# saamiya225/Graph-and-sequential-recommendation-systems

Measured on AMD Instinct MI355X. Metric: BPR training steps/sec (one step = K-layer LightGCN propagation + BPR loss + backward + Adam on a global batch of 2048 triplets), higher is better.
Workload: dtype bf16 (activation storage; f32 accumulation, parameters, gradients and Adam); 1 GPU; gowalla: 29858 users x 40981 items, 810128 train interactions, nnz(A_hat)=1620256, layers=3, dim=64, bpr_batch=2048; global_batch=2048, per_gpu_batch=2048, scaling_mode=strong, multi_gpu_status=n/a, parallelism=single GPU, act_dtype=bf16, xcd_remap=1, row_order=xcd

## Files before the change

graph-and-sequential-recommendation-systems_amd/_lib.py:

```python
import ctypes as C
import os

from . import build as _build

F32, BF16, FP8 = 0, 1, 2
ABI_VERSION = 13
MAX_LAYERS = 8
MAX_NEG_RATIO = 16

LOSS_BPR, LOSS_SOFTMAX, LOSS_INBATCH = 0, 1, 2
LOSS_DIRECTAU = 4
SCORE_DOT, SCORE_COSINE = 0, 1

_c_i32p =C.POINTER(C.c_int32)
_c_i64p = C.POINTER(C.c_int64)
_c_f32p = C.POINTER(C.c_float)
_vp = C.c_void_p


def fp8_col_of_byte(d):
    import numpy as np
    b = np.arange(d)
    l, j, e = b // 16, (b % 16) // 4, b % 4
    return ((j * (d // 16) + l) * 4 + e).astype(np.int64)
# ... 65 lines not shown
    "lgcn_ctx_get_step": (C.c_int64, [_vp]),
    "lgcn_ctx_hub_rows": (C.c_int64, [_vp]),
    "lgcn_ctx_set_step": (None, [_vp, C.c_int64]),
    "lgcn_ctx_set_lr": (None, [_vp, C.c_double]),
    "lgcn_ctx_set_dp_local": (C.c_int, [_vp, C.c_int]),
    "lgcn_train_step": (C.c_int, [_vp, _vp, _vp, _vp, C.c_int32, _vp, _vp]),
    "lgcn_train_epoch": (C.c_int, [_vp, _vp, _vp, _vp, C.c_int64, C.c_int32, _vp, _vp]),
    "lgcn_apply_perm_multi": (C.c_int, [_vp, C.c_int, _vp, C.c_int64, _vp, _vp, _vp, C.c_int32, _vp]),
    "lgcn_train_step_multi": (C.c_int, [_vp, _vp, _vp, _vp, C.c_int64, C.c_int32, C.c_int32, _vp, _vp]),
    "lgcn_train_epoch_multi": (C.c_int, [_vp, _vp, _vp, _vp, C.c_int32, C.c_int64, C.c_int32, _vp, _vp]),
    "lgcn_ctx_set_loss": (C.c_int, [_vp, C.c_int32, C.c_float]),
    "lgcn_ctx_get_loss": (C.c_int32, [_vp, _vp]),
    "lgcn_train_step_inbatch": (C.c_int, [_vp, _vp, _vp, C.c_int32, _vp, _vp]),
    "lgcn_train_epoch_inbatch": (C.c_int, [_vp, _vp, _vp, C.c_int64, C.c_int32, _vp, _vp]),
    "lgcn_ctx_set_inbatch_scores": (C.c_int, [_vp, C.c_int, _vp]),
    "lgcn_ctx_get_inbatch_scores": (C.c_int, [_vp, C.POINTER(_vp)]),
    "lgcn_ctx_set_inbatch_mix": (C.c_int, [_vp, C.c_int32]),
    "lgcn_ctx_get_inbatch_mix": (C.c_int32, [_vp]),
    "lgcn_train_step_inbatch_mix": (C.c_int, [_vp, _vp, _vp, _vp, C.c_int64, C.c_int32, C.c_int32, _vp, _vp]),
    "lgcn_train_epoch_inbatch_mix": (C.c_int, [_vp, _vp, _vp, _vp, C.c_int32, C.c_int64, C.c_int32, _vp, _vp]),
    "lgcn_ctx_set_directau": (C.c_int, [_vp, C.c_float]),
    "lgcn_ctx_get_directau": (C.c_int, [_vp, _vp]),
    "lgcn_train_step_directau": (C.c_int, [_vp, _vp, _vp, C.c_int32, _vp, _vp]),
    "lgcn_train_epoch_directau": (C.c_int, [_vp, _vp, _vp, C.c_int64, C.c_int32, _vp, _vp]),
    "lgcn_ctx_set_hard_neg": (C.c_int, [_vp, C.c_int32, C.c_uint64, _vp]),
    "lgcn_ctx_get_hard_neg": (C.c_int32, [_vp]),
    "lgcn_hard_neg_rank": (C.c_uint32, [C.c_uint64, C.c_int64, C.c_int32, C.c_int32]),
    "lgcn_dp_block_floats": (C.c_int64, [_vp, C.c_int32, C.c_int32]),
    "lgcn_train_step_dp_part1": (C.c_int, [_vp, _vp, _vp, _vp, C.c_int32, C.c_int32, C.c_int32, _vp]),
    "lgcn_train_step_dp_dense_part1": (C.c_int, [_vp, _vp, _vp, _vp, C.c_int32, C.c_int32, C.c_int32, _vp]),
    "lgcn_ctx_gate_total": (C.c_int, [_vp, C.POINTER(C.c_void_p), C.POINTER(C.c_int32)]),
    "lgcn_train_step_dp_part2": (C.c_int, [_vp, _vp, _vp, _vp, C.c_int32, C.c_int32, _vp, _vp, _vp]),
    "lgcn_ctx_check": (C.c_int, [_vp, _vp]),
    "lgcn_eval_topk": (C.c_int, [_vp, C.c_int32, C.c_int32, C.c_int32, _vp, C.c_int32, _vp, _vp, C.c_int32, _vp, _vp, _vp]),
    "lgcn_eval_topk_masked": (C.c_int, [_vp, C.c_int32, C.c_int32, C.c_int32, _vp, C.c_int32, _vp, _vp, C.c_int32, _vp, _vp, _vp, _vp]),
    "lgcn_eval_mask_words": (C.c_int64, [C.c_int32, C.c_int32]),
    "lgcn_eval_build_masks": (C.c_int, [_vp, C.c_int32, _vp, _vp, C.c_int32, _vp, _vp]),
    "lgcn_eval_topk_fp32": (C.c_int, [_vp, C.c_int32, C.c_int32, C.c_int32, _vp, C.c_int32, _vp, _vp, C.c_int32, _vp, _vp, _vp]),
    "lgcn_eval_metrics": (C.c_int, [_vp, C.c_int32, C.c_int32, _vp, _vp, _vp, C.c_int32, _vp, _vp, _vp]),
    "lgcn_eval_kmax": (C.c_int32, []),
    "lgcn_eval_topk_ex": (C.c_int, [_vp, C.c_int32, C.c_int32, C.c_int32, _vp, C.c_int32, _vp, _vp, _vp, C.c_int32, _vp, _vp,
                                    C.c_int64, C.c_int32, _vp]),
    "lgcn_eval_metrics_ex": (C.c_int, [_vp, C.c_int32, C.c_int32, _vp, _vp, _vp, C.c_int32, _vp, _vp, _vp]),
    "lgcn_eval_ranks": (C.c_int, [_vp, C.c_int32, C.c_int32, C.c_int32, _vp, C.c_int32, _vp, _vp, _vp, _vp, C.c_int64, _vp, _vp, _vp,
                                  C.c_int32, _vp]),
    "lgcn_eval_rank_metrics": (C.c_int, [C.c_int32, C.c_int32, _vp, _vp, _vp, _vp, _vp, C.c_int64, _vp, _vp, _vp, _vp, C.c_int32,
                                         _vp, _vp, _vp]),
    "lgcn_i2i_topk": (C.c_int, [_vp, _vp, C.c_int64, C.c_int64, C.c_int32, C.c_int32, C.c_int32, C.c_int32, _vp, _vp, _vp, _vp]),
    "lgcn_i2i_finish": (C.c_int, [_vp, _vp, _vp, C.c_int32, C.c_int32, C.c_int64, _vp, _vp, _vp, C.POINTER(C.c_int64), _vp]),
    "lgcn_dp_available": (C.c_int, []),
    "lgcn_dp_unique_id": (C.c_int, [_vp]),
    "lgcn_dp_init": (C.c_int, [_vp, C.c_int, C.c_int, C.POINTER(_vp)]),
    "lgcn_train_step_i64": (C.c_int, [_vp, _vp, _vp, _vp, C.c_int32, _vp, _vp, _vp]),
    "lgcn_train_step_cols_part1": (C.c_int, [_vp, _vp, _vp, _vp, C.c_int32, C.POINTER(_vp), _vp]),
    "lgcn_train_step_cols_part2": (C.c_int, [_vp, _vp, _vp, _vp, C.c_int32, _vp, _vp]),
    "lgcn_dp_allreduce_sum_f32": (C.c_int, [_vp, _vp, C.c_int64, _vp]),
    "lgcn_dp_init_loopback": (C.c_int, [C.c_int, C.POINTER(_vp)]),
    "lgcn_dp_destroy": (None, [_vp]),
    "lgcn_dp_world": (C.c_int, [_vp]),
    "lgcn_dp_rank": (C.c_int, [_vp]),
    "lgcn_train_epoch_dp": (C.c_int, [_vp, _vp, _vp, _vp, _vp, C.c_int64, C.c_int32, C.c_int32, _vp, _vp, _vp, _vp]),
    "lgcn_rs_phase": (C.c_int, [_vp, C.c_int32, C.c_int32, _vp, _vp, _vp, C.c_int32, C.c_int32, C.c_int32, _vp, _vp, _vp]),
    "lgcn_rs_buffer": (C.c_int, [_vp, C.c_int32, C.c_int32, C.POINTER(_vp), C.POINTER(C.c_int32)]),
    "lgcn_ctx_set_dropout": (C.c_int, [_vp, C.c_float, C.c_uint64]),
    "lgcn_ctx_set_layer_weights": (C.c_int, [_vp, _vp, C.c_int32]),
    "lgcn_ctx_get_layer_weights": (C.c_int32, [_vp, _vp]),
    "lgcn_propagate_weighted": (C.c_int, [_vp, _vp, C.c_int, C.c_int, C.c_int, _vp, _vp, _vp, _vp]),
    "lgcn_dropout_mask": (C.c_int, [_vp, _vp, C.c_int64, C.c_int64, C.c_float, C.c_uint64, C.c_int64, _vp, _vp]),
    "lgcn_spmm_csr_drop": (C.c_int, [_vp, _vp, C.c_int, _vp, C.c_int, C.c_int, C.c_float, C.c_uint64, C.c_int64, C.c_int, _vp]),
    "lgcn_mf_create": (C.c_int, [C.POINTER(MfConfig), C.POINTER(_vp)]),
    "lgcn_mf_destroy": (None, [_vp]),
    "lgcn_mf_get_step": (C.c_int64, [_vp]),
    "lgcn_mf_set_step": (None, [_vp, C.c_int64]),
    "lgcn_mf_set_lr": (None, [_vp, C.c_double]),
    "lgcn_mf_train_step": (C.c_int, [_vp, _vp, _vp, _vp, C.c_int32, _vp, _vp]),
    "lgcn_mf_train_epoch": (C.c_int, [_vp, _vp, _vp, _vp, C.c_int64, C.c_int32, _vp, _vp]),
    "lgcn_mf_check": (C.c_int, [_vp, _vp]),
    "lgcn_ctx_set_fold_g32": (C.c_int, [_vp, C.c_int]),
    "lgcn_ctx_folded_steps": (C.c_int64, [_vp]),
    "lgcn_ctx_copy_arrivals": (C.c_int, [_vp, _vp, C.c_int64]),
    "lgcn_slot_multiplicity": (C.c_int, [_vp, _vp, _vp, C.c_int64, C.c_int32, C.c_int32, C.c_int64, _vp, _vp]),
    "lgcn_ctx_set_store_policy": (C.c_int, [_vp, C.c_int]),
    "lgcn_ctx_get_store_policy": (C.c_int, [_vp, _c_i32p]),
}

STORE_ADAM, STORE_XLAST = 1, 2
STORE_ARG_MV, STORE_ARG_P, STORE_ARG_Y = 1, 2, 4

_LIB = None


class LgcnError(RuntimeError):
    pass


def load():
    global _LIB
    if _LIB is not None:
        return _LIB
    path = _build.LIB_PATH
    if os.environ.get("LGCN_LIB_PATH"):
        pass
    elif _build.is_stale():
        if _build.must_not_build():
            if not os.path.exists(path):
                raise LgcnError(
                    f"liblgcn_hip.so is missing at {path}; this process is a distributed rank or runs under a "
                    "profiler and will not compile it. Build it first (__graft_entry__.build()).")
        elif _build.find_hipcc() is not None:
            _build.build()
        elif not os.path.exists(path):
            raise LgcnError(
                f"liblgcn_hip.so is missing at {path} and hipcc is not available to build it. "
                "The MI355X HIP library is the product path; there is no CPU fallback.")
    try:
        lib = C.CDLL(path)
    except OSError as e:
        raise LgcnError(f"cannot load {path}: {e}") from e
    for name, (res, args) in SIGNATURES.items():
        try:
            fn = getattr(lib, name)
        except AttributeError as e:
            raise LgcnError(f"{path} does not export {name} (stale build?)") from e
        fn.restype, fn.argtypes = res, args
    if lib.lgcn_abi_version() != ABI_VERSION:
        raise LgcnError("liblgcn_hip.so ABI version mismatch")
    _LIB = lib
    return lib


def check(rc, what=""):
    if rc != 0:
        msg = load().lgcn_last_error()
        raise LgcnError(f"{what} failed (rc={rc}): {msg.decode() if msg else ''}")


def npp(a):
    return a.ctypes.data_as(_vp)


def tp(t):
    return _vp(t.data_ptr()) if t is not None else _vp(0)


def require_gpu():
    import torch
    if not torch.cuda.is_available() or not load().lgcn_device_available():
        raise LgcnError("no MI355X/HIP device visible: the LightGCN HIP kernels cannot run "
                        "(there is deliberately no CPU fallback)")


def current_stream():
    import torch
    return _vp(torch.cuda.current_stream().cuda_stream)


EVAL_FP32 = 1


def eval_kmax():
    return int(load().lgcn_eval_kmax())


def _want(t, name, dtype, shape, dev=None):
    import torch
    if not torch.is_tensor(t):
        raise ValueError(f"{name} must be a tensor")
    if t.dtype != dtype:
# ... 321 lines not shown
```

graph-and-sequential-recommendation-systems_amd/csrc/lgcn_device.hip:

```cpp
#include <hip/hip_runtime.h>
#include <stdint.h>
#include <stdio.h>
#include <math.h>

#include "lgcn_device_common.h"

typedef __attribute__((ext_vector_type(8))) float f32x8;
typedef __attribute__((ext_vector_type(4))) __bf16 bf16x4;
typedef __attribute__((ext_vector_type(8))) __bf16 bf16x8;
typedef __attribute__((ext_vector_type(16))) float f32x16;
typedef __attribute__((ext_vector_type(16))) __bf16 bf16x16;
typedef __attribute__((ext_vector_type(4))) uint32_t u32x4;
typedef __attribute__((ext_vector_type(2))) float f32x2;
struct fp8_t { uint8_t v; };
__host__ __device__ __forceinline__ int fp8_byte_of_col(int c, int D) { const int L = D / 16, q = c >> 2; return (q % L) * 16 + 4 * (q / L) + (c & 3); }
__device__ __forceinline__ const float *fp8_scales(const void *tab, int64_t n_rows, int D) { return (const float *)((const char *)tab + n_rows * D); }
__device__ __forceinline__ float *fp8_scales(void *tab, int64_t n_rows, int D) { return (float *)((char *)tab + n_rows * D); }

template <int C> struct VecF;
template <> struct VecF<4> { typedef f32x4 T; typedef bf16x4 B; };
template <> struct VecF<8> { typedef f32x8 T; typedef bf16x8 B; };
template <> struct VecF<16> { typedef f32x16 T; typedef bf16x16 B; };

template <int C> __device__ __forceinline__ typename VecF<C>::T zerov() {
    typename VecF<C>::T z;
#pragma unroll
    for (int i = 0; i < C; i++) z[i] = 0.f;
    return z;
}
template <int C> __device__ __forceinline__ typename VecF<C>::T loadv(const float *p) {
    return *reinterpret_cast<const typename VecF<C>::T *>(p);
}
template <int C> __device__ __forceinline__ typename VecF<C>::T loadv(const bf16_t *p) {
    return __builtin_convertvector(*reinterpret_cast<const typename VecF<C>::B *>(p), typename VecF<C>::T);
}
template <int C> __device__ __forceinline__ void storev(float *p, typename VecF<C>::T v) {
    *reinterpret_cast<typename VecF<C>::T *>(p) = v;
}
template <int C> __device__ __forceinline__ void storev(bf16_t *p, typename VecF<C>::T v) {
    *reinterpret_cast<typename VecF<C>::B *>(p) = __builtin_convertvector(v, typename VecF<C>::B);
}
__device__ __forceinline__ f32x4 load4(const float *p) { return loadv<4>(p); }
__device__ __forceinline__ f32x4 load4(const bf16_t *p) { return loadv<4>(p); }
__device__ __forceinline__ void store4(float *p, f32x4 v) { storev<4>(p, v); }
__device__ __forceinline__ void store4(bf16_t *p, f32x4 v) { storev<4>(p, v); }
template <int OFF> __device__ __forceinline__ void store16_wt(void *p, f32x4 v) {
    static_assert(OFF >= 0 && OFF < 4096 && OFF % 16 == 0, "immediate offset of a global store");
    asm volatile("global_store_dwordx4 %0, %1, off offset:%2 sc1\n\ts_nop 1" : : "v"(p), "v"(v), "n"(OFF) : "memory");
}
template <int C> __device__ __forceinline__ void storev_wt(float *p, typename VecF<C>::T v) {
    store16_wt<0>(p, f32x4{v[0], v[1], v[2], v[3]});
    if constexpr (C >= 8) store16_wt<16>(p, f32x4{v[4], v[5], v[6], v[7]});
    if constexpr (C == 16) { store16_wt<32>(p, f32x4{v[8], v[9], v[10], v[11]}); store16_wt<48>(p, f32x4{v[12], v[13], v[14], v[15]}); }
}
__device__ __forceinline__ void storev_wt(bf16_t *p, f32x8 v) {
    union { bf16x8 b; f32x4 f; } u; u.b = __builtin_convertvector(v, bf16x8);
    store16_wt<0>(p, u.f);
}
__device__ __forceinline__ float fp8_decode(uint8_t b) { return __builtin_amdgcn_cvt_pk_f32_fp8((int)b, false)[0]; }
template <> __device__ __forceinline__ float tab_elem<fp8_t>(const void *tab, int64_t n_rows, int D, int64_t row, int col) {
    return fp8_scales(tab, n_rows, D)[row] * fp8_decode(((const uint8_t *)tab)[row * D + fp8_byte_of_col(col, D)]);
}
__device__ __forceinline__ void fp8_row_scale(float amax, float &scale, float &inv) {
    const uint32_t E = __float_as_uint(amax) >> 23;
    if (E < 27u || E == 255u) { scale = 1.f; inv = E == 255u ? 1.f : 0.f; return; }
    scale = __uint_as_float((E - 6u) << 23); inv = __uint_as_float((260u - E) << 23);
}
template <int D, int C, bool IL>
__device__ __forceinline__ void store_row_fp8(void *tab, int64_t n_rows, int64_t row, int l, typename VecF<C>::T v) {
    static_assert(!IL || C == 16, "interleaved accumulators come from fp8 gathers: 16 per lane");
    constexpr int LPR = D / C;
    float amax = 0.f;
#pragma unroll
    for (int i = 0; i < C; i++) amax = fmaxf(amax, fabsf(v[i]));
#pragma unroll
    for (int o = 1; o < LPR; o <<= 1) amax = fmaxf(amax, __shfl_xor(amax, o));
    float scale, inv;
    fp8_row_scale(amax, scale, inv);
    uint32_t w[C / 4];
#pragma unroll
    for (int i = 0; i < C / 4; i++) {
        int p = 0;
        p = __builtin_amdgcn_cvt_pk_fp8_f32(v[4 * i] * inv, v[4 * i + 1] * inv, p, false);
        p = __builtin_amdgcn_cvt_pk_fp8_f32(v[4 * i + 2] * inv, v[4 * i + 3] * inv, p, true);
        w[i] = (uint32_t)p;
    }
    if (IL) {
        uint32_t *dst = (uint32_t *)((char *)tab + row * D + l * 16);
#pragma unroll
        for (int i = 0; i < C / 4; i++) dst[i] = w[i];
    } else {
#pragma unroll
        for (int i = 0; i < C / 4; i++) *(uint32_t *)((char *)tab + row * D + fp8_byte_of_col((l * (C / 4) + i) * 4, D)) = w[i];
    }
    if (l == 0) fp8_scales(tab, n_rows, D)[row] = scale;
}
template <int D, int C, bool IL> __device__ __forceinline__ typename VecF<C>::T row_load(const float *base, int64_t row, int l) {
    if constexpr (!IL) return loadv<C>(base + row * D + l * C);
    else {
        typename VecF<C>::T r;
#pragma unroll
        for (int j = 0; j < 4; j++) {
            const f32x4 t = load4(base + row * D + (j * (D / 16) + l) * 4);
            r[4 * j] = t.x; r[4 * j + 1] = t.y; r[4 * j + 2] = t.z; r[4 * j + 3] = t.w;
        }
        return r;
    }
}
template <int D, int C, bool IL> __device__ __forceinline__ void row_store(float *base, int64_t row, int l, typename VecF<C>::T v, bool wt = false) {
    if constexpr (!IL) {
        if (wt) storev_wt<C>(base + row * D + l * C, v);
        else storev<C>(base + row * D + l * C, v);
    } else if (wt) {
        float *p = base + row * D + l * 4;
        store16_wt<0>(p, f32x4{v[0], v[1], v[2], v[3]}); store16_wt<D>(p, f32x4{v[4], v[5], v[6], v[7]});
        store16_wt<2 * D>(p, f32x4{v[8], v[9], v[10], v[11]}); store16_wt<3 * D>(p, f32x4{v[12], v[13], v[14], v[15]});
    } else {
#pragma unroll
        for (int j = 0; j < 4; j++) store4(base + row * D + (j * (D / 16) + l) * 4, f32x4{v[4 * j], v[4 * j + 1], v[4 * j + 2], v[4 * j + 3]});
    }
}
template <int D, int C, typename TO, bool IL> struct RowStore {
    static __device__ __forceinline__ void put(void *Y, int64_t, int64_t row, int l, typename VecF<C>::T v, bool wt = false) {
        static_assert(!IL, "an fp8 gather writes fp32 or fp8");
        if constexpr (C == 8) { if (wt) { storev_wt((TO *)Y + row * D + l * C, v); return; } }
        storev<C>((TO *)Y + row * D + l * C, v); }
};
template <int D, int C, bool IL> struct RowStore<D, C, float, IL> {
    static __device__ __forceinline__ void put(void *Y, int64_t, int64_t row, int l, typename VecF<C>::T v, bool wt = false) { row_store<D, C, IL>((float *)Y, row, l, v, IL ? false : wt); }
};
template <int D, int C, bool IL> struct RowStore<D, C, fp8_t, IL> {
    static __device__ __forceinline__ void put(void *Y, int64_t n_rows, int64_t row, int l, typename VecF<C>::T v, bool = false) { store_row_fp8<D, C, IL>(Y, n_rows, row, l, v); }
};
__device__ __forceinline__ bool bit_set(const uint32_t *bm, int i) { return (bm[i >> 5] >> (i & 31)) & 1u; }

template <int C> __device__ __forceinline__ typename VecF<C>::T loadv_fixed(const long long *p, float div) {
// ... 122 lines not shown
}
__device__ __forceinline__ float sum_xor16(float v) {
    typedef __attribute__((ext_vector_type(2))) unsigned u32x2;
    const unsigned a = __float_as_uint(v);
    const u32x2 r = __builtin_amdgcn_permlane16_swap(a, a, false, false);
    return __uint_as_float(r.x) + __uint_as_float(r.y);
}
template <int ROT> __device__ __forceinline__ float sum_ror(float v) {
    return v + __int_as_float(__builtin_amdgcn_update_dpp(0, __float_as_int(v), 0x120 + ROT, 0xf, 0xf, false));
}
template <int LPR, typename Acc>
__device__ __forceinline__ Acc reduce_groups(Acc acc) {
    constexpr int C = sizeof(Acc) / sizeof(float);
#pragma unroll
    for (int i = 0; i < C; i++) {
        float v = acc[i];
        if (LPR <= 32) v = sum_xor32(v);
        if (LPR <= 16) v = sum_xor16(v);
        if (LPR <= 8) v = sum_ror<8>(v);
        if (LPR <= 4) v = sum_ror<4>(v);
        acc[i] = v;
    }
    return acc;
}

struct CsrSrc {
    const int32_t *indices; const float *vals;
    __device__ __forceinline__ int2 at(int64_t i) const { return make_int2(indices[i], __float_as_int(vals[i])); }
};
struct PackedSrc {
    const int2 *pk;
    __device__ __forceinline__ int2 at(int64_t i) const { return pk[i]; }
};

__device__ __forceinline__ bool drop_apply(const DropArgs &d, int row, int2 &cv) {
    const bool live = drop_live(d, row, cv.x);
    cv.y = live ? __float_as_int(__int_as_float(cv.y) * d.inv) : 0;
    return live;
}

template <int D, typename TI, bool SPARSE, bool BIG, bool DROP = false, typename ES>
__device__ __forceinline__ typename Geo<D, TI, SPARSE>::Acc
row_gather(const ES &es, int64_t start, int64_t end, const GatherSrc &src, int lane, int2 *stage, int row = 0) {
    typedef Geo<D, TI, SPARSE> G;
    typename G::Acc acc = zerov<G::CPL>();
    tile_pad_init(stage, lane);
    int2 cv = make_int2(0, 0);
    if (start + lane < end) cv = es.at(start + lane);
    for (int64_t base = start; base < end; base += 64) {
        const int n = (int)min((int64_t)64, end - base);
        if (!SPARSE && src.S) cv.y = __float_as_int(__int_as_float(cv.y) * src.S[cv.x]);
        bool live = true;
        if constexpr (DROP) live = drop_apply(src.dr, row, cv);
        const int cnt = tile_stage<SPARSE>(cv.x, __int_as_float(cv.y), n, src, lane, stage, live);
        __builtin_amdgcn_wave_barrier();
        cv = make_int2(0, 0);
        if (base + 64 + lane < end) cv = es.at(base + 64 + lane);
        tile_gather<D, TI, SPARSE, BIG>(stage, cnt, src, lane, acc);
        __builtin_amdgcn_wave_barrier();
    }
    return reduce_groups<G::LPR>(acc);
}

template <int C> struct AdamPre { typename VecF<C>::T p, m, v; bool have; };

template <int D, typename TO, int MODE, int C, bool IL = false>
__device__ __forceinline__ void spmm_epilogue(const SpmmArgs &a, int64_t row, int l, typename VecF<C>::T acc, bool flagged,
                                              const AdamPre<C> *pre = nullptr) {
    typedef typename VecF<C>::T V;
    const int64_t off = row * D + l * C;
    if (MODE & M_ADDSELF) acc = row_load<D, C, IL>(a.selfX, row, l) + acc;
    if (MODE & M_WTS) acc = a.w_in * acc;
    if ((MODE & M_ADDG) && flagged) {
        V g = row_load<D, C, IL>(a.G32, row, l);
        if (MODE & M_WTS) g = a.w_add * g;
        acc = g + acc;
        if ((MODE & M_ADAM) && !(MODE & M_SPARSE) && a.clear) {
            if constexpr (IL) {
#pragma unroll
                for (int j = 0; j < 4; j++) {
                    i64x2 *q = reinterpret_cast<i64x2 *>(a.G64 + row * D + (j * (D / 16) + l) * 4);
                    q[0] = i64x2{0, 0}; q[1] = i64x2{0, 0};
                }
            } else {
                i64x2 *q = reinterpret_cast<i64x2 *>(a.G64 + off);
#pragma unroll
                for (int i = 0; i < C / 2; i++) q[i] = i64x2{0, 0};
            }
        }
    }
    if (MODE & M_ADAM) {
        V p, m, v;
        if (pre && pre->have) { p = pre->p; m = pre->m; v = pre->v; }
        else { p = row_load<D, C, IL>(a.P, row, l); m = row_load<D, C, IL>(a.M, row, l); v = row_load<D, C, IL>(a.V, row, l); }
        if ((MODE & M_ADDG) && a.cnt && flagged) {
            const int n_slots = a.cnt[row];
            acc = acc + (a.lam * (float)n_slots) * p;
            if (l == 0) a.cnt[row] = 0;
        }
        m = m + a.w1 * (acc - m);
        v = v * a.beta2 + (a.omb2 * acc) * acc;
        V denom;
#pragma unroll
        for (int i = 0; i < C; i++) denom[i] = sqrtf(v[i]) / a.bc2_sqrt + a.eps;
        p = p - a.step_size * (m / denom);
        row_store<D, C, IL>(a.P, row, l, p, (a.wt & LGCN_STORE_ARG_P) != 0);
        row_store<D, C, IL>(a.M, row, l, m, (a.wt & LGCN_STORE_ARG_MV) != 0); row_store<D, C, IL>(a.V, row, l, v, (a.wt & LGCN_STORE_ARG_MV) != 0);
        if constexpr (!(MODE & M_SPARSE)) {
            if (a.Pb) storev<C>(a.Pb + off, p);
            if (a.Pq) store_row_fp8<D, C, IL>(a.Pq, a.n_rows, row, l, p);
        }
    } else {
        RowStore<D, C, TO, IL>::put(a.Y, a.n_rows, row, l, acc, (a.wt & LGCN_STORE_ARG_Y) != 0);
    }
}

__device__ __forceinline__ void reduce_loss_wave(const float *terms, const float *gathered, int B, int shard,
                                                 int D, float decay, float *loss_out, int lane, float ent_coeff = 0.f, int64_t blk_in = 0) {
    float fl = 0.f, fr = 0.f, fe = 0.f;
    if (ent_coeff != 0.f) {
        if (!gathered) { for (int b = lane; b < B; b += 64) fe += terms[2 * B + b]; }
        else for (int b = lane; b < B; b += 64) fe += gathered[(int64_t)(b / shard) * blk_in + (int64_t)3 * shard * D + 2 * shard + b % shard];
    }
    if (!gathered) {
#pragma unroll 8
        for (int b = lane; b < B; b += 64) { fl += terms[b]; fr += terms[B + b]; }
    } else {
        constexpr int UL = 16;
        const int64_t blk = blk_in ? blk_in : (int64_t)3 * shard * D + 2 * shard;
        int r = lane / shard, i = lane % shard;
        for (int b0 = 0; b0 < B; b0 += 64 * UL) {
            float tl[UL], tr[UL];
#pragma unroll
            for (int u = 0; u < UL; u++) {
                const bool in = b0 + u * 64 + lane < B;
                const float *t = gathered + (in ? r : 0) * blk + (int64_t)3 * shard * D;
                const int ii = in ? i : 0;
                tl[u] = t[ii]; tr[u] = t[shard + ii];
                i += 64;
                while (i >= shard) { i -= shard; r++; }
            }
#pragma unroll
            for (int u = 0; u < UL; u++) {
                const bool in = b0 + u * 64 + lane < B;
                fl += in ? tl[u] : 0.f; fr += in ? tr[u] : 0.f;
            }
        }
    }
#pragma unroll
    for (int off = 32; off > 0; off >>= 1) { fl += __shfl_xor(fl, off); fr += __shfl_xor(fr, off); fe += __shfl_xor(fe, off); }
    if (lane == 0) {
        const float bpr = -(fl / (float)B) - ent_coeff * (fe / (float)(2 * B));
        const float reg = (0.5f * fr) / (float)B;
        loss_out[0] = bpr + decay * reg; loss_out[1] = bpr; loss_out[2] = reg;
    }
}

#ifndef SPMM_MIN_WAVES
#define SPMM_MIN_WAVES 6
#endif
#ifndef SPMM_MIN_WAVES_ADAM
#define SPMM_MIN_WAVES_ADAM 5
#endif
#ifndef SPMM_ADAM_PREFETCH
#define SPMM_ADAM_PREFETCH 1
#endif
#ifndef SPMM_U_SP
#define SPMM_U_SP 4
#endif
#ifndef SPMM_U
#define SPMM_U 8
#endif
template <int D, typename TI, bool SPARSE, int U, int GPR, bool PRE, bool BIG, int PC>
__device__ __forceinline__ void pack_batch(const int2 *p, const GatherSrc &src, int l,
                                           typename Geo<D, TI, SPARSE>::Acc &acc,
                                           const SpmmArgs *a, int64_t off, bool final_batch,
                                           AdamPre<PC> *pre) {
    typedef Raw<TI, SPARSE> R;
    int2 cv[U]; typename R::T xr[U];
#pragma unroll
    for (int u = 0; u < U; u++) cv[u] = p[u * GPR];
#pragma unroll
    for (int u = 0; u < U; u++) xr[u] = R::template load<BIG>(src, cv[u].x, D, l);
    if (PRE && final_batch && off >= 0) {
        pre->p = loadv<PC>(a->P + off); pre->m = loadv<PC>(a->M + off); pre->v = loadv<PC>(a->V + off);
        pre->have = true;
    }
    __builtin_amdgcn_sched_barrier(0);
#pragma unroll
    for (int u = 0; u < U; u++) acc += __int_as_float(cv[u].y) * R::cvt(xr[u], src.div);
}

#ifndef SPMM_WAVE_ROWS
#define SPMM_WAVE_ROWS 1
#endif
#ifndef SPMM_WPB
#define SPMM_WPB 1
#endif
template <int NPW> struct PackGeo { static constexpr int PACKS = NPW >= SPMM_WAVE_ROWS ? 1 : SPMM_WAVE_ROWS / NPW, RPW = NPW * PACKS, RPB = SPMM_WPB * RPW; };
#ifndef SPMM_GPR_BF16
#define SPMM_GPR_BF16 2
#endif
#ifndef SPMM_SCALAR_ROWINFO
#define SPMM_SCALAR_ROWINFO 1
#endif
#ifndef SPMM_ADAM_SPLIT
#define SPMM_ADAM_SPLIT 1
#endif
#ifndef SPMM_ADAM_PREFETCH_BF16
#define SPMM_ADAM_PREFETCH_BF16 0
#endif
#ifndef SPMM_GPR_F32
#define SPMM_GPR_F32 1
#endif
template <int D, typename TI, bool SP> struct RowGeo {
    static constexpr int NPW = Geo<D, TI, SP>::NPW;
    static constexpr int WANT = SP ? 1 : (Geo<D, TI, SP>::CPL == 16 ? (NPW >= 4 ? NPW / 4 : 1) : Geo<D, TI, SP>::CPL == 8 ? SPMM_GPR_BF16 : SPMM_GPR_F32);
    static constexpr int GPR = NPW >= WANT ? WANT : NPW;
    static constexpr int RPK = NPW / GPR;
};
template <int O> __device__ __forceinline__ float sum_xor(float v, int lane) {
    if (O == 32) return sum_xor32(v);
    if (O == 16) return sum_xor16(v);
    if (O == 8) return sum_ror<8>(v);
    const float dn = __int_as_float(__builtin_amdgcn_update_dpp(0, __float_as_int(v), 0x120 + 4, 0xf, 0xf, false));
    const float up = __int_as_float(__builtin_amdgcn_update_dpp(0, __float_as_int(v), 0x120 + 12, 0xf, 0xf, false));
    return v + ((lane & 4) ? dn : up);
}
template <int LPR, int GPR> __device__ __forceinline__ float sum_row_groups(float v, int lane) {
    if (GPR >= 2) v = sum_xor<LPR>(v, lane);
    if (GPR >= 4) v = sum_xor<(2 * LPR > 32 ? 32 : 2 * LPR)>(v, lane);
    return v;
}

template <int D, typename TI, typename TO, int MODE, bool BIG, bool DROP = false>
__global__ void __launch_bounds__(64 * SPMM_WPB, sizeof(TI) == 1 ? 4 : ((MODE & M_ADAM) && sizeof(TI) == 4) ? SPMM_MIN_WAVES_ADAM : SPMM_MIN_WAVES) k_spmm(SpmmArgs a) {
    constexpr bool SP = (MODE & M_SPARSE) != 0;
    typedef Geo<D, TI, SP> G;
    typedef typename G::Acc Acc;
    typedef Raw<TI, SP> R;
    constexpr int LPR = G::LPR, NPW = G::NPW, C = G::CPL;
    constexpr bool IL = !SP && sizeof(TI) == 1;
    constexpr int GPR = RowGeo<D, TI, SP>::GPR, RPK = RowGeo<D, TI, SP>::RPK;
    static_assert(GPR == 1 || GPR == 2 || GPR == 4, "one, two or four lane groups per row");
    static_assert(LPR * GPR <= 64 && (GPR == 1 || LPR >= 4), "lane groups of a row must fit the wave");
    constexpr int PACKS = PackGeo<RPK>::PACKS, RPW = PackGeo<RPK>::RPW, RPB = PackGeo<RPK>::RPB;
    constexpr int ST = 76;
    static_assert(64 + 3 * GPR <= ST, "staged row + padding");
    constexpr int U = SP ? SPMM_U_SP : (C == 16 ? 4 : SPMM_U);
    __shared__ int2 stage_lds[SPMM_WPB][(RPK * ST > TILE_ST ? RPK * ST : TILE_ST)];
    const int lane = threadIdx.x & 63;
    const int wid = __builtin_amdgcn_readfirstlane(threadIdx.x >> 6);
    GatherSrc src;
    src.X = SP ? (const void *)a.G32 : a.X; src.bm = a.bitmap; src.div = a.div;
    src.S = (!SP && sizeof(TI) == 1) ? fp8_scales(a.X, a.n_rows, D) : nullptr;
    if constexpr (DROP) src.dr = a.dr;
    if ((MODE & M_ADAM) && !SP && a.clear && blockIdx.x == 0 && wid == SPMM_WPB - 1)
        reduce_loss_wave(a.terms, a.gathered, a.B, a.shard, D, a.decay, a.loss_out, lane, a.ent_coeff, a.blk);
    int x, j;
    if (a.remap) { x = blockIdx.x & (XCDS - 1); j = blockIdx.x >> 3; }
    else {
        x = 0; j = blockIdx.x;
        while (x < XCDS - 1) {
            const int nb = (a.sp.cblk[x + 1] - a.sp.cblk[x]) * (4 / SPMM_WPB) + (a.sp.rows[x + 1] - a.sp.rows[x]) / RPB;
            if (j < nb) break;
            j -= nb; x++;
        }
    }
    const int ncb = (a.sp.cblk[x + 1] - a.sp.cblk[x]) * (4 / SPMM_WPB);
    if (j < ncb) {
        const int c = a.sp.cblk[x] * 4 + j * SPMM_WPB + wid;
#if SPMM_SCALAR_ROWINFO
        typedef int i32x4c_ __attribute__((ext_vector_type(4)));
        const i32x4c_ chv = ((const __attribute__((address_space(4))) i32x4c_ *)a.lp.chunks)[c];
        const int4 ch = make_int4(chv.x, chv.y, chv.z, chv.w);
        const int o = ch.x;
        if (o < 0) return;
        const int64_t row = ((const __attribute__((address_space(4))) int32_t *)a.lp.long_row)[o];
        const int nch = ((const __attribute__((address_space(4))) int32_t *)a.lp.long_nch)[o];
        const bool rflag = (MODE & M_ADDG) ? ((((const __attribute__((address_space(4))) uint32_t *)a.bitmap)[row >> 5] >> (row & 31)) & 1u) != 0u : false;
#else
        const int4 ch = a.lp.chunks[c];
        const int o = ch.x;
        if (o < 0) return;
        const int64_t row = a.lp.long_row[o];
        const int nch = a.lp.long_nch[o];
        const bool rflag = (MODE & M_ADDG) ? bit_set(a.bitmap, (int)row) : false;
#endif
        Acc acc = row_gather<D, TI, SP, BIG, DROP>(PackedSrc{a.pk}, ch.y, ch.z, src, lane, stage_lds[wid], (int)row);
        if (nch == 1) {
            if (lane < LPR) spmm_epilogue<D, TO, MODE, C, IL>(a, row, lane, acc, rflag);
            return;
        }
        typedef __attribute__((address_space(1))) unsigned long long gu64;
        if (lane < LPR) {
            union { Acc v; unsigned long long q[C / 2]; } pk; pk.v = acc;
            gu64 *dst = (gu64 *)(a.lp.partials + (int64_t)c * D + lane * C);
#pragma unroll
            for (int i = 0; i < C / 2; i++) __hip_atomic_store(dst + i, pk.q[i], __ATOMIC_RELAXED, __HIP_MEMORY_SCOPE_AGENT);
        }
        asm volatile("s_waitcnt vmcnt(0)" ::: "memory");
        int ticket = 0;
        if (lane == 0) ticket = __hip_atomic_fetch_add(a.lp.counters + o, 1, __ATOMIC_RELAXED, __HIP_MEMORY_SCOPE_AGENT);
        ticket = __builtin_amdgcn_readfirstlane(ticket);
        if (ticket != nch - 1) return;
        __builtin_amdgcn_fence(__ATOMIC_ACQUIRE, "agent");
        asm volatile("s_waitcnt vmcnt(0)" ::: "memory");
        if (lane == 0) __hip_atomic_store(a.lp.counters + o, 0, __ATOMIC_RELAXED, __HIP_MEMORY_SCOPE_AGENT);
        if (lane >= LPR) return;
        const int first = c - ch.w;
        Acc tot = zerov<C>();
        for (int k = 0; k < nch; k++) {
            union { Acc v; unsigned long long q[C / 2]; } pk;
            gu64 *sp_ = (gu64 *)(a.lp.partials + (int64_t)(first + k) * D + lane * C);
#pragma unroll
            for (int i = 0; i < C / 2; i++) pk.q[i] = __hip_atomic_load(sp_ + i, __ATOMIC_RELAXED, __HIP_MEMORY_SCOPE_AGENT);
            if (k == 0) tot = pk.v; else tot += pk.v;
        }
        spmm_epilogue<D, TO, MODE, C, IL>(a, row, lane, tot, rflag);
        return;
    }
    const int t = j - ncb;
    if (t >= (a.sp.rows[x + 1] - a.sp.rows[x]) / RPB) return;
    const int g = lane / LPR, l = lane % LPR;
    int2 *stage = stage_lds[wid];
#pragma unroll 1
    for (int pk = 0; pk < PACKS; pk++) {
        const int64_t pos0 = (int64_t)a.sp.rows[x] + (int64_t)t * RPB + (wid * PACKS + pk) * RPK;
        int off[RPK + 1];
        off[0] = 0;
#if SPMM_SCALAR_ROWINFO
        typedef int i32x4_ __attribute__((ext_vector_type(4)));
        typedef const __attribute__((address_space(4))) i32x4_ *kint4p;
        typedef const __attribute__((address_space(4))) uint32_t *ku32p;
        const kint4p rip = (kint4p)(a.rowinfo + pos0);
        int row_s[RPK];
        int64_t base = 0;
#pragma unroll
        for (int r = 0; r < RPK; r++) {
            const i32x4_ ri = rip[r];
            row_s[r] = ri.x; off[r + 1] = off[r] + ri.z;
            if (r == 0) base = ri.y;
        }
        if (row_s[0] < 0) break;
        uint32_t fw_s[RPK];
#pragma unroll
        for (int r = 0; r < RPK; r++) fw_s[r] = ((MODE & M_ADDG) && row_s[r] >= 0) ? ((ku32p)a.bitmap)[row_s[r] >> 5] : 0u;
        const int tot = off[RPK];
#else
        int my_row = -1, my_s = 0, my_n = 0;
        if (lane < RPK) {
            const int4 ri = a.rowinfo[pos0 + lane];
            my_row = ri.x; my_s = ri.y; my_n = ri.z;
        }
        uint32_t my_fw = 0u;
        if ((MODE & M_ADDG) && my_row >= 0) my_fw = a.bitmap[my_row >> 5];
        if (__builtin_amdgcn_readlane(my_row, 0) < 0) break;
#pragma unroll
        for (int r = 0; r < RPK; r++) off[r + 1] = off[r] + __builtin_amdgcn_readlane(my_n, r);
        const int tot = off[RPK];
        const int64_t base = __builtin_amdgcn_readlane(my_s, 0);
#endif
        int2 cvr[RPK];
#pragma unroll
        for (int it = 0; it < RPK; it++) {
            cvr[it] = make_int2(0, 0);
            if (it * 64 < tot) { const int e = it * 64 + lane; if (e < tot) cvr[it] = a.pk[base + e]; }
        }
        const int myr = g / GPR, sub = g % GPR;
        int maxcnt = 0;
        if (!SP && sizeof(TI) == 1) {
#pragma unroll
            for (int it = 0; it < RPK; it++)
                if (it * 64 < tot) cvr[it].y = __float_as_int(__int_as_float(cvr[it].y) * src.S[cvr[it].x]);
        }
        bool live[RPK];
#pragma unroll
        for (int it = 0; it < RPK; it++) live[it] = true;
        if constexpr (DROP) {
#pragma unroll
            for (int it = 0; it < RPK; it++) {
                if (it * 64 < tot) {
                    const int e = it * 64 + lane;
#if SPMM_SCALAR_ROWINFO
                    int rid = row_s[0];
#pragma unroll
                    for (int k = 1; k < RPK; k++) rid = (e >= off[k]) ? row_s[k] : rid;
#else
                    int r = 0;
#pragma unroll
                    for (int k = 1; k < RPK; k++) r += (e >= off[k]) ? 1 : 0;
// ... 646 lines not shown
            if (lane < Hg) DH[sidx * GATE_HMAX + lane] = HR[sidx * GATE_HMAX + lane] > 0.f ? dlogit * V2[lane] : 0.f;
            if (lane == 0) DLOG[sidx] = dlogit;
            __builtin_amdgcn_wave_barrier();
#pragma unroll
            for (int j = 0; j < CPT; j++) {
                const int c = j * LPT + lane;
                float die = 0.f, dip = 0.f;
                if (col) {
#pragma unroll 8
                    for (int k = 0; k < Hg; k++) { const float dh = DH[sidx * GATE_HMAX + k]; die += V1p[k * V1S + c] * dh; dip += V1p[k * V1S + D + c] * dh; }
                }
                const float de = g[q] * dF[j] + die, dpv = (1.f - g[q]) * dF[j] + dip;
                if (col) {
                    DPV[sidx * D + c] = dpv;
                    if (a.G64) fixed_add(a.G64 + row * D + c, de);
                    if (a.exchange) a.contrib[((int64_t)(1 + q) * a.shard + b) * D + c] = de;
                }
            }
            if (a.G64 && lane == 0) {
                atomicOr(a.bitmap + (row >> 5), 1u << (row & 31));
                if (a.item_bitmap) atomicOr(a.item_bitmap + (item[q] >> 5), 1u << (item[q] & 31));
            }
            __builtin_amdgcn_wave_barrier();
            if (lane < Hp) {
                float da = 0.f;
#pragma unroll 16
                for (int c = 0; c < D; c++) da += W2p[c * W2S + lane] * DPV[sidx * D + c];
                DA[sidx * GATE_HMAX + lane] = AA[sidx * GATE_HMAX + lane] > 0.f ? da : 0.f;
            }
        }
    }
    __syncthreads();
    long long *out = a.partials + (int64_t)blockIdx.x * a.P;
    auto fx = [](float v) { return __double2ll_rn((double)v * FIXED_SCALE); };
#define GATE_SUM(EXPR) _Pragma("unroll") for (int w2 = 0; w2 < GATE_S; w2 += 2) { float pr_; { const int sI = w2; pr_ = (EXPR); } { const int sI = w2 + 1; pr_ += (EXPR); } v += fx(pr_); }
    for (int i = tid; i < a.P; i += 256) {
        long long v = 0;
        if (i < Hp) { GATE_SUM(DA[sI * GATE_HMAX + i] * SC[sI]) }
        else if (i < oW2) { const int k = i - Hp; GATE_SUM(DA[sI * GATE_HMAX + k]) }
        else if (i < ob2) { const int c = (i - oW2) / Hp, k = (i - oW2) % Hp; GATE_SUM(DPV[sI * D + c] * AA[sI * GATE_HMAX + k]) }
        else if (i < oV1) { const int c = i - ob2; GATE_SUM(DPV[sI * D + c]) }
        else if (i < oc1) { const int jj = (i - oV1) / D2, c = (i - oV1) % D2; GATE_SUM(DH[sI * GATE_HMAX + jj] * IN[sI * D2 + c]) }
        else if (i < oV2) { const int jj = i - oc1; GATE_SUM(DH[sI * GATE_HMAX + jj]) }
        else if (i < oc2) { const int jj = i - oV2; GATE_SUM(DLOG[sI] * HR[sI * GATE_HMAX + jj]) }
        else { GATE_SUM(DLOG[sI]) }
        out[i] = v;
    }
#undef GATE_SUM
}
static size_t gate_lds_bytes(int D) {
    const size_t fl = (size_t)GATE_HMAX * (2 * D + 1) + (size_t)D * (GATE_HMAX + 1) + 2 * GATE_HMAX + D + 2 * GATE_HMAX
                    + (size_t)GATE_S * 2 * D + 2 * GATE_S * GATE_HMAX + (size_t)GATE_S * D + 2 * GATE_S * GATE_HMAX + 2 * GATE_S;
    return fl * sizeof(float);
}
int lgcn_gate_launch(const GateArgs &g, int d, hipStream_t st) {
    const unsigned grid = (unsigned)((g.B + GATE_TPB - 1) / GATE_TPB);
    const size_t lds = gate_lds_bytes(d);
    switch (d) {
    case 32: HIP_OK(hipFuncSetAttribute((const void *)k_triplet_gate<32>, hipFuncAttributeMaxDynamicSharedMemorySize, (int)lds));
             hipLaunchKernelGGL((k_triplet_gate<32>), dim3(grid), dim3(256), lds, st, g); break;
    case 64: HIP_OK(hipFuncSetAttribute((const void *)k_triplet_gate<64>, hipFuncAttributeMaxDynamicSharedMemorySize, (int)lds));
             hipLaunchKernelGGL((k_triplet_gate<64>), dim3(grid), dim3(256), lds, st, g); break;
    case 128: HIP_OK(hipFuncSetAttribute((const void *)k_triplet_gate<128>, hipFuncAttributeMaxDynamicSharedMemorySize, (int)lds));
             hipLaunchKernelGGL((k_triplet_gate<128>), dim3(grid), dim3(256), lds, st, g); break;
    default: lgcn_set_error("popularity gate: embedding dim must be 32, 64 or 128"); return 3;
    }
    return 0;
}

__global__ void __launch_bounds__(256) k_gate_adam(GateAdamArgs a) {
    const int i = blockIdx.x * 256 + threadIdx.x;
    if (i >= a.P) return;
    long long q = 0;
    for (int q0 = 0; q0 < a.n_src; q0 += 32) {
        long long t[32];
#pragma unroll
        for (int u = 0; u < 32; u++) t[u] = q0 + u < a.n_src ? a.src[(int64_t)(q0 + u) * a.stride + i] : 0;
#pragma unroll
        for (int u = 0; u < 32; u++) q += t[u];
    }
    const float g = (float)((double)q * FIXED_INV);
    a.grad_out[i] = g;
    float m = a.m[i], v = a.v[i], p = a.params[i];
    m = m + a.w1 * (g - m);
    v = v * a.beta2 + (a.omb2 * g) * g;
    const float denom = sqrtf(v) / a.bc2_sqrt + a.eps;
    p = p - a.step_size * (m / denom);
    a.params[i] = p; a.m[i] = m; a.v[i] = v;
}
__global__ void __launch_bounds__(256) k_gate_rank_total(const long long *partials, int32_t n_part, int32_t P, long long *out) {
    const int i = blockIdx.x * 256 + threadIdx.x;
    if (i >= P) return;
    long long q = 0;
    for (int w = 0; w < n_part; w++) q += partials[(int64_t)w * P + i];
    out[i] = q;
}
void lgcn_gate_adam_launch(const GateAdamArgs &a, hipStream_t st) {
    hipLaunchKernelGGL(k_gate_adam, dim3((unsigned)((a.P + 255) / 256)), dim3(256), 0, st, a);
}
void lgcn_gate_rank_total_launch(const long long *partials, int32_t n_part, int32_t P, long long *out, hipStream_t st) {
    hipLaunchKernelGGL(k_gate_rank_total, dim3((unsigned)((P + 255) / 256)), dim3(256), 0, st, partials, n_part, P, out);
}

template <typename TI>
__global__ void __launch_bounds__(256) k_mean_layers(MeanSplitArgs a) {
    const float div = (float)(a.K + 1);
    for (int64_t i = (int64_t)blockIdx.x * 256 + threadIdx.x; i < a.n4; i += (int64_t)gridDim.x * 256) {
        f32x4 s = load4(a.X0 + i * 4);
        for (int k = 1; k <= a.K; k++) s += load4((const TI *)a.Xl[k] + i * 4);
        store4((i < a.n4_users ? a.out_u : a.out_i) + i * 4, s / div);
    }
}
__global__ void __launch_bounds__(256) k_flag_range(uint32_t *bm, int64_t lo, int64_t hi) {
    const int64_t wlo = lo >> 5, whi = (hi + 31) >> 5;
    for (int64_t wd = wlo + (int64_t)blockIdx.x * 256 + threadIdx.x; wd < whi; wd += (int64_t)gridDim.x * 256) {
        uint32_t m = 0xffffffffu;
        if (wd == (lo >> 5)) m &= 0xffffffffu << (lo & 31);
        if (wd == (hi >> 5)) m &= (hi & 31) ? (0xffffffffu >> (32 - (hi & 31))) : 0u;
        if (m == 0xffffffffu) bm[wd] = m; else if (m) atomicOr(bm + wd, m);
    }
}
void lgcn_mean_layers_launch(const MeanSplitArgs &m, int act_dtype, hipStream_t st) {
    const int64_t blocks = (m.n4 + 255) / 256;
    const unsigned grid = (unsigned)(blocks < 2048 ? blocks : 2048);
    if (act_dtype == LGCN_F32) hipLaunchKernelGGL((k_mean_layers<float>), dim3(grid), dim3(256), 0, st, m);
    else hipLaunchKernelGGL((k_mean_layers<bf16_t>), dim3(grid), dim3(256), 0, st, m);
}
void lgcn_flag_range_launch(uint32_t *bm, int64_t lo, int64_t hi, hipStream_t st) {
    const int64_t words = (hi + 31) / 32;
    hipLaunchKernelGGL(k_flag_range, dim3((unsigned)((words + 255) / 256 < 64 ? (words + 255) / 256 : 64)), dim3(256), 0, st, bm, lo, hi);
}

__device__ __forceinline__ int64_t slot_row(int c, int b, const int32_t *users, const int32_t *pos,
                                            const int32_t *neg, int32_t n_users, int64_t N) {
    const int u = users[b], p = pos[b], n = neg[b];
    if (u < 0 || u >= n_users || p < 0 || (int64_t)p + n_users >= N || n < 0 || (int64_t)n + n_users >= N) return -1;
    return c == 0 ? (int64_t)u : (int64_t)(c == 1 ? p : n) + n_users;
}

template <int D>
__global__ void __launch_bounds__(256) k_scatter(SlotArgs a) {
    constexpr int LPT = D < 64 ? D : 64, CPT = D / LPT, SPB = 256 / LPT;
    const int s = blockIdx.x * SPB + threadIdx.x / LPT, l = threadIdx.x % LPT;
    if (s >= 3 * a.B) return;
    const int c = s / a.B, b = s % a.B;
    const int64_t row = slot_row(c, b, a.users, a.pos, a.neg, a.n_users, a.N);
    if (row < 0) return;
    const int r = b / a.shard, i = b % a.shard;
    if (r == a.skip_rank) return;
    const int64_t blk = a.blk ? a.blk : (int64_t)3 * a.shard * D + 2 * a.shard;
    const float *src = a.gathered + r * blk + ((int64_t)c * a.shard + i) * D;
#pragma unroll
    for (int j = 0; j < CPT; j++)
        fixed_add(a.G64 + row * D + j * LPT + l, src[j * LPT + l]);
    if (l == 0) {
        atomicOr(a.bitmap + (row >> 5), 1u << (row & 31));
        if (a.cnt) atomicAdd(a.cnt + row, 1);
        if (a.item_bitmap && c > 0) { const int64_t it = row - a.n_users; atomicOr(a.item_bitmap + (it >> 5), 1u << (it & 31)); }
    }
}

template <int D>
__global__ void __launch_bounds__(256) k_g32(SlotArgs a) {
    constexpr int LPR = D / 4, SPB = 256 / LPR;
    const int s = blockIdx.x * SPB + threadIdx.x / LPR, l = threadIdx.x % LPR;
    if (s >= 3 * a.B) return;
    const int64_t row = slot_row(s / a.B, s % a.B, a.users, a.pos, a.neg, a.n_users, a.N);
    if (row < 0) return;
    store4(a.G32 + row * D + l * 4, loadv_fixed<4>(a.G64 + row * D + l * 4, a.div));
}

// ... 316 lines not shown
```

graph-and-sequential-recommendation-systems_amd/csrc/lgcn_device_common.h:

```cpp
#ifndef LGCN_DEVICE_COMMON_H
#define LGCN_DEVICE_COMMON_H
#include <hip/hip_runtime.h>
#include <math.h>
#include <stdint.h>
#include <stdio.h>

#include "lgcn_hip.h"
#include "lgcn_internal.h"

#define FIXED_SCALE 1125899906842624.0
#define FIXED_INV   8.8817841970012523e-16

typedef __attribute__((ext_vector_type(4))) float f32x4;
typedef __attribute__((ext_vector_type(2))) long long i64x2;

#define DISPATCH_D(d, ...)                                                       \
    switch (d) {                                                                 \
    case 32: { constexpr int D = 32; __VA_ARGS__; } break;                       \
    case 64: { constexpr int D = 64; __VA_ARGS__; } break;                       \
    case 128: { constexpr int D = 128; __VA_ARGS__; } break;                     \
    case 256: { constexpr int D = 256; __VA_ARGS__; } break;                     \
    default: lgcn_set_error("embedding dim must be 32, 64, 128 or 256"); return 3; \
    }

__device__ __forceinline__ float logsigmoid_f(float x) { return fminf(x, 0.f) - log1pf(expf(-fabsf(x))); }
__device__ __forceinline__ float sigmoid_neg_f(float x) {
    const float z = expf(-fabsf(x));
    return x < 0.f ? 1.f / (1.f + z) : z / (1.f + z);
}

template <typename TI> __device__ __forceinline__ float tab_at(const void *tab, int64_t o) { return (float)((const TI *)tab)[o]; }
template <typename TI> __device__ __forceinline__ float tab_elem(const void *tab, int64_t n_rows, int D, int64_t row, int col);
template <> __device__ __forceinline__ float tab_elem<float>(const void *tab, int64_t, int D, int64_t row, int col) { return tab_at<float>(tab, row * D + col); }
template <> __device__ __forceinline__ float tab_elem<bf16_t>(const void *tab, int64_t, int D, int64_t row, int col) { return tab_at<bf16_t>(tab, row * D + col); }

template <int LPT> __device__ __forceinline__ float group_sum(float v) {
#pragma unroll
    for (int off = 1; off < LPT; off <<= 1) v += __shfl_xor(v, off);
    return v;
}
template <int LPT> __device__ __forceinline__ float group_max(float v) {
#pragma unroll
    for (int off = 1; off < LPT; off <<= 1) v = fmaxf(v, __shfl_xor(v, off));
    return v;
}

template <int D, typename TI, bool WTS>
__device__ __forceinline__ void slot_row(const MultiNegArgs &a, int64_t row, int l, float *e, float *e0) {
    constexpr int LPT = D < 64 ? D : 64, CPT = D / LPT;
    const float div = (float)(a.K + 1);
#pragma unroll
    for (int j = 0; j < CPT; j++) {
        const int64_t o = row * D + j * LPT + l;
        float s = a.X0[o];
        e0[j] = s;
        if constexpr (WTS) {
            s *= a.w[0];
            for (int k = 1; k <= a.K; k++) s += a.w[k] * tab_at<TI>(a.Xl[k], o);
            e[j] = s;
        } else {
            for (int k = 1; k <= a.K; k++) s += tab_at<TI>(a.Xl[k], o);
            e[j] = s / div;
        }
    }
}

__device__ __forceinline__ void fixed_add(long long *g64, float g) {
    atomicAdd((unsigned long long *)g64, (unsigned long long)__double2ll_rn((double)g * FIXED_SCALE));
}
#endif
```

graph-and-sequential-recommendation-systems_amd/csrc/lgcn_kernels.h:

```cpp
#ifndef LGCN_KERNELS_H
#define LGCN_KERNELS_H
#include <hip/hip_runtime.h>
#include <stdint.h>

#include "lgcn_hip.h"

typedef __bf16 bf16_t;

#ifndef LGCN_GATHER_U
#define LGCN_GATHER_U 8
#endif

struct DropArgs { uint32_t k0, k1, thr; float inv; int32_t tr; int32_t on; };

#define LONG_T 64
#define SLICE_PAD 64
#ifndef SHORT_WIN
#define SHORT_WIN 2048
#endif
#ifndef LONG_CH
#define LONG_CH 512
#endif
#define XCDS 8
struct LongPlan {
    const int4 *chunks;
    const int32_t *long_row;
    const int32_t *long_nch;
    float *partials;
    int32_t *counters;
    int32_t n_long, n_chunk_slots;
};
struct SlicePlan {
    int32_t cblk[XCDS + 1];
    int32_t rows[XCDS + 1];
};

struct SpmmArgs {
    const int2 *pk;
    const int4 *rowinfo;
    LongPlan lp; SlicePlan sp;
    const void *X; void *Y;
    int64_t n_rows;
    long long *G64; uint32_t *bitmap; float div;
    const float *G32;
    float *P; float *M; float *V;
    bf16_t *Pb;
    void *Pq;
    int clear;
    const float *terms; const float *gathered; float *loss_out; int32_t B, shard; float decay;
    float ent_coeff;
    int64_t blk;
    float step_size, bc2_sqrt, w1, beta2, omb2, eps;
    int remap;
    const float *selfX;
    int32_t *cnt; float lam;
    DropArgs dr;
    float w_in, w_add;
    int32_t wt;
};

enum { M_SPARSE = 1, M_ADDG = 2, M_ADAM = 4, M_ADDSELF = 8, M_WTS = 16 };

int lgcn_spmm_launch(const SpmmArgs &a, int mode, int d, int x_dtype, int y_dtype, hipStream_t st);

struct MeanArgs {
    const float *X0; const void *Xl[LGCN_MAX_LAYERS + 1]; int K;
    float *out; int64_t n4;
    int32_t d; int64_t N;
    float w[LGCN_MAX_LAYERS + 1];
};
void lgcn_layer_mean_launch(const MeanArgs &m, int act_dtype, bool wts, hipStream_t st);

void lgcn_to_bf16_launch(const float *src, bf16_t *dst, int64_t n, hipStream_t st);
int lgcn_to_fp8_launch(const float *src, void *dst, int64_t n_rows, int d, hipStream_t st);

#ifndef TRIPLET_HUB_NNZ
#define TRIPLET_HUB_NNZ 131072
#endif
#ifndef TRIPLET_HUB_CHUNK
#define TRIPLET_HUB_CHUNK 2048
#endif
struct BprArgs {
    const int32_t *indptr; const int32_t *indices; const float *vals;
    const float *X0; const void *Xl[LGCN_MAX_LAYERS + 1]; int K;
    int32_t n_users; int64_t N;
    const int32_t *users; const int32_t *pos; const int32_t *neg;
    int32_t B_local;
    int32_t shard;
    float inv_B;
    float lam;
    long long *G64;
    uint32_t *bitmap;
    uint32_t *stale_bitmap; int64_t bitmap_words;
    uint32_t *item_bitmap;
    float *contrib;
    int32_t exchange;
    const float *Xhub; int32_t hub_nnz;
    float *terms;
    int32_t terms_off, terms_stride;
    int32_t *err;
    int32_t dense_last;
    int32_t reg_ego;
    int32_t *cnt;
    int32_t cols_phase; float *erows; float *colsum;
    DropArgs dr;
    float w[LGCN_MAX_LAYERS + 1];
    const uint16_t *mult; float *G32; float gdiv; int32_t *arrive;
};
int lgcn_triplet_launch(const BprArgs &a, int d, int act_dtype, bool wts, bool big, hipStream_t st);

#define GATE_TPB 8
#define GATE_HMAX 64
struct GateArgs {
    const float *E;
    const float *item_pop;
    const float *params;
    long long *partials;
    int32_t Hp, Hg, P;
    float inv_temp, ent_scale;
    int32_t n_users; int64_t N;
    const int32_t *users; const int32_t *pos; const int32_t *neg;
    int32_t B; float inv_B, lam;
    long long *G64; uint32_t *bitmap; uint32_t *item_bitmap;
    uint32_t *stale_bitmap; int64_t bitmap_words;
    float *terms; int32_t terms_stride;
    int32_t *err;
    float *contrib; int32_t shard; int32_t exchange;
};
int lgcn_gate_launch(const GateArgs &g, int d, hipStream_t st);
void lgcn_gate_rank_total_launch(const long long *partials, int32_t n_part, int32_t P, long long *out, hipStream_t st);
struct GateAdamArgs {
    const long long *src; int32_t n_src; int64_t stride; int32_t P;
    float *params, *m, *v, *grad_out;
    float step_size, bc2_sqrt, w1, beta2, omb2, eps;
};
void lgcn_gate_adam_launch(const GateAdamArgs &a, hipStream_t st);

struct MeanSplitArgs {
    const float *X0; const void *Xl[LGCN_MAX_LAYERS + 1]; int K;
    float *out_u, *out_i; int64_t n4_users, n4;
};
void lgcn_mean_layers_launch(const MeanSplitArgs &m, int act_dtype, hipStream_t st);
void lgcn_flag_range_launch(uint32_t *bm, int64_t lo, int64_t hi, hipStream_t st);

struct SlotArgs {
    const int32_t *users; const int32_t *pos; const int32_t *neg;
    int32_t B; int32_t n_users; int64_t N;
    long long *G64; uint32_t *bitmap;
    float *G32; float div;
    const float *gathered; int32_t shard; int32_t world;
    int32_t skip_rank;
    const float *terms; float *loss_out; float decay;
    float ent_coeff;
    int64_t blk;
    uint32_t *item_bitmap;
    int32_t *cnt;
};
int lgcn_scatter_launch(const SlotArgs &s, int d, hipStream_t st);
int lgcn_g32_launch(const SlotArgs &s, int d, hipStream_t st);
int lgcn_finish_launch(const SlotArgs &s, int d, hipStream_t st);
void lgcn_flag_rows_launch(const SlotArgs &s, hipStream_t st);
struct SlotArgsMulti {
    SlotArgs s;
    const int32_t *negs; int64_t neg_stride; int32_t R;
};
int lgcn_g32_multi_launch(const SlotArgsMulti &s, int d, hipStream_t st);
int lgcn_finish_multi_launch(const SlotArgsMulti &s, int d, hipStream_t st);

#define SLOT_MULT_HMAX 16384
#define SLOT_MULT_THREADS 1024
struct SlotMultArgs {
    const int32_t *users; const int32_t *pos; const int32_t *neg;
    int64_t T; int32_t B; int32_t n_users; int64_t N;
    uint16_t *out; int32_t H;
};
static inline int32_t slot_mult_hash(int32_t B) {
    if (B <= 0) return 0;
    int64_t H = 64;
    while (3 * H < 12 * (int64_t)B) H <<= 1;
    return H <= SLOT_MULT_HMAX ? (int32_t)H : 0;
}
int lgcn_slot_mult_launch(const int32_t *users, const int32_t *pos, const int32_t *neg, int64_t T, int32_t B, int32_t n_users,
                          int64_t N, uint16_t *out, hipStream_t st);

void lgcn_apply_perm_launch(const int32_t *S, int cols, const int64_t *perm, int64_t T, int32_t *users, int32_t *pos, int32_t *neg,
                            hipStream_t st);
void lgcn_apply_perm_multi_launch(const int32_t *S, int cols, const int64_t *perm, int64_t T, int32_t *users, int32_t *pos,
                                  int32_t *negs, int32_t R, hipStream_t st);

void lgcn_index_range_launch(const int32_t *indices, int64_t nnz, int32_t n_rows, int32_t *bad);
void lgcn_pack_stream_launch(const int4 *items, int64_t n_items, const int32_t *indices, const float *vals, int2 *pk);
void lgcn_dropout_mask_launch(const int32_t *indptr, const int32_t *indices, int64_t n_rows, int64_t nnz, uint32_t k0, uint32_t k1,
                              uint64_t thr, uint8_t *keep_out, hipStream_t st);
#endif
```

graph-and-sequential-recommendation-systems_amd/csrc/lgcn_mf.hip:

```cpp
#include <new>

#include "lgcn_device_common.h"

#define MF_ADAM_BLOCKS_MAX 16384

struct lgcn_mf {
    lgcn_mf_config c;
    int64_t N;
    int64_t bm_words;
    int64_t step;
    int flip;
};

template <int CTRL> __device__ __forceinline__ float mf_add_dpp(float v) {
    return v + __int_as_float(__builtin_amdgcn_update_dpp(0, __float_as_int(v), CTRL, 0xf, 0xf, false));
}
template <int G> __device__ __forceinline__ float mf_group_sum(float v) {
    typedef __attribute__((ext_vector_type(2))) unsigned u32x2;
    v = mf_add_dpp<0xB1>(v);
    v = mf_add_dpp<0x4E>(v);
    v = mf_add_dpp<0x141>(v);
    if (G >= 16) v = mf_add_dpp<0x140>(v);
    if (G >= 32) { const unsigned a = __float_as_uint(v); const u32x2 r = __builtin_amdgcn_permlane16_swap(a, a, false, false); v = __uint_as_float(r.x) + __uint_as_float(r.y); }
    if (G >= 64) { const unsigned a = __float_as_uint(v); const u32x2 r = __builtin_amdgcn_permlane32_swap(a, a, false, false); v = __uint_as_float(r.x) + __uint_as_float(r.y); }
    return v;
}

struct MfTripletArgs {
    const float *E;
    const int32_t *users, *pos, *neg;
    int32_t B, n_users, m_items;
    float decay, Bf;
    long long *G64; uint32_t *bitmap;
    float *terms;
    int32_t *err;
};

template <int D>
__global__ void __launch_bounds__(256) k_mf_triplet(MfTripletArgs a) {
    constexpr int G = D / 4, TPB = 256 / G;
    const int l = (int)threadIdx.x % G;
    const int64_t b = (int64_t)blockIdx.x * TPB + (int)threadIdx.x / G;
    const bool in = b < a.B;
    int32_t iu = 0, ip = 0, in_ = 0;
    if (in) { iu = a.users[b]; ip = a.pos[b]; in_ = a.neg[b]; }
    const bool bad = in && (iu < 0 || iu >= a.n_users || ip < 0 || ip >= a.m_items || in_ < 0 || in_ >= a.m_items);
    const bool ok = in && !bad;
    const int64_t ru = (int64_t)iu, rp = (int64_t)ip + a.n_users, rn = (int64_t)in_ + a.n_users;
    f32x4 u = {0.f, 0.f, 0.f, 0.f}, p = u, n = u;
    if (ok) {
        u = *reinterpret_cast<const f32x4 *>(a.E + ru * D + 4 * l);
        p = *reinterpret_cast<const f32x4 *>(a.E + rp * D + 4 * l);
        n = *reinterpret_cast<const f32x4 *>(a.E + rn * D + 4 * l);
    }
    float ps = 0.f, ns = 0.f, rr = 0.f;
#pragma unroll
    for (int i = 0; i < 4; i++) { ps += u[i] * p[i]; ns += u[i] * n[i]; rr += u[i] * u[i] + p[i] * p[i] + n[i] * n[i]; }
    ps = mf_group_sum<G>(ps); ns = mf_group_sum<G>(ns); rr = mf_group_sum<G>(rr);
    if (!in) return;
    if (bad) {
        if (l == 0) { atomicExch(a.err, 1); a.terms[b] = 0.f; a.terms[a.B + b] = 0.f; }
        return;
    }
    const float x = ns - ps;
    const float e = expf(-fabsf(x));
    const float s = (x >= 0.f ? 1.f : e) / (1.f + e);
    if (l == 0) {
        a.terms[b] = fmaxf(x, 0.f) + log1pf(e);
        a.terms[a.B + b] = rr;
    }
    long long *gu = a.G64 + ru * D + 4 * l, *gp = a.G64 + rp * D + 4 * l, *gn = a.G64 + rn * D + 4 * l;
#pragma unroll
    for (int i = 0; i < 4; i++) {
        const float du = (s * (n[i] - p[i]) + a.decay * u[i]) / a.Bf;
        const float dp = (a.decay * p[i] - s * u[i]) / a.Bf;
        const float dn = (s * u[i] + a.decay * n[i]) / a.Bf;
        fixed_add(gu + i, du);
        fixed_add(gp + i, dp);
        fixed_add(gn + i, dn);
    }
    if (l == 0) {
        atomicOr(a.bitmap + (ru >> 5), 1u << (ru & 31));
        atomicOr(a.bitmap + (rp >> 5), 1u << (rp & 31));
        atomicOr(a.bitmap + (rn >> 5), 1u << (rn & 31));
    }
}

struct MfAdamArgs {
    float *P, *M, *V;
    long long *G64; const uint32_t *bitmap;
    uint32_t *stale_bitmap; int64_t bitmap_words;
    int64_t n_vec;
    const float *terms; float *loss_out; int32_t B; float decay;
    float step_size, bc2_sqrt, w1, beta2, omb2, eps;
};

__device__ __forceinline__ void mf_reduce_loss_wave(const MfAdamArgs &a, int lane) {
    float fl = 0.f, fr = 0.f;
#pragma unroll 8
    for (int b = lane; b < a.B; b += 64) { fl += a.terms[b]; fr += a.terms[a.B + b]; }
#pragma unroll
    for (int off = 32; off > 0; off >>= 1) { fl += __shfl_xor(fl, off); fr += __shfl_xor(fr, off); }
    if (lane == 0) {
        const float bpr = fl / (float)a.B;
        const float reg = (0.5f * fr) / (float)a.B;
        a.loss_out[0] = bpr + a.decay * reg; a.loss_out[1] = bpr; a.loss_out[2] = reg;
    }
}

template <int D>
__global__ void __launch_bounds__(256) k_mf_adam(MfAdamArgs a) {
    if (blockIdx.x == gridDim.x - 1) {
        if (threadIdx.x < 64) mf_reduce_loss_wave(a, (int)threadIdx.x);
        return;
    }
    constexpr int G = D / 4;
    const int64_t stride = (int64_t)(gridDim.x - 1) * 256;
    const int64_t t0 = (int64_t)blockIdx.x * 256 + threadIdx.x;
    for (int64_t i = t0; i < a.bitmap_words; i += stride) a.stale_bitmap[i] = 0u;
    for (int64_t i = t0; i < a.n_vec; i += stride) {
        const int64_t row = i / G;
        const uint32_t word = a.bitmap[row >> 5];
        f32x4 p = *reinterpret_cast<const f32x4 *>(a.P + 4 * i);
        f32x4 m = *reinterpret_cast<const f32x4 *>(a.M + 4 * i);
        f32x4 v = *reinterpret_cast<const f32x4 *>(a.V + 4 * i);
        f32x4 g = {0.f, 0.f, 0.f, 0.f};
        if ((word >> (row & 31)) & 1u) {
            i64x2 *q = reinterpret_cast<i64x2 *>(a.G64 + 4 * i);
            const i64x2 q0 = q[0], q1 = q[1];
            g[0] = (float)((double)q0.x * FIXED_INV); g[1] = (float)((double)q0.y * FIXED_INV);
            g[2] = (float)((double)q1.x * FIXED_INV); g[3] = (float)((double)q1.y * FIXED_INV);
            q[0] = i64x2{0, 0}; q[1] = i64x2{0, 0};
        }
        m = m + a.w1 * (g - m);
        v = v * a.beta2 + (a.omb2 * g) * g;
        f32x4 denom;
#pragma unroll
        for (int k = 0; k < 4; k++) denom[k] = sqrtf(v[k]) / a.bc2_sqrt + a.eps;
        p = p - a.step_size * (m / denom);
        *reinterpret_cast<f32x4 *>(a.P + 4 * i) = p;
        *reinterpret_cast<f32x4 *>(a.M + 4 * i) = m;
        *reinterpret_cast<f32x4 *>(a.V + 4 * i) = v;
    }
}

extern "C" int lgcn_mf_create(const lgcn_mf_config *cfg, lgcn_mf **out) {
    if (!cfg || !out) { lgcn_set_error("lgcn_mf_create: null argument"); return 3; }
    const lgcn_mf_config &c = *cfg;
    if (c.d != 32 && c.d != 64 && c.d != 128 && c.d != 256) { lgcn_set_error("lgcn_mf_create: d must be 32, 64, 128 or 256"); return 3; }
    if (c.n_users <= 0 || c.m_items <= 0) { lgcn_set_error("lgcn_mf_create: n_users and m_items must be positive"); return 3; }
    if ((int64_t)c.n_users + (int64_t)c.m_items >= ((int64_t)1 << 31)) { lgcn_set_error("lgcn_mf_create: n_users + m_items must stay below 2^31"); return 3; }
    if (c.max_batch < 1) { lgcn_set_error("lgcn_mf_create: max_batch must be at least 1"); return 3; }
    if (!c.E0 || !c.adam_m || !c.adam_v || !c.G64 || !c.bitmap || !c.terms || !c.err) { lgcn_set_error("lgcn_mf_create: null buffer"); return 3; }
    lgcn_mf *x = new (std::nothrow) lgcn_mf();
    if (!x) { lgcn_set_error("lgcn_mf_create: out of host memory"); return 4; }
    x->c = c; x->N = (int64_t)c.n_users + c.m_items; x->bm_words = (x->N + 31) / 32; x->step = 0; x->flip = 0;
    *out = x;
    return 0;
}

extern "C" void lgcn_mf_destroy(lgcn_mf *mf) { delete mf; }
extern "C" int64_t lgcn_mf_get_step(const lgcn_mf *mf) { return mf ? mf->step : -1; }
extern "C" void lgcn_mf_set_step(lgcn_mf *mf, int64_t step) { if (mf) mf->step = step; }
extern "C" void lgcn_mf_set_lr(lgcn_mf *mf, double lr) { if (mf) mf->c.lr = lr; }

static int mf_check_batch(const lgcn_mf *x, const void *u, const void *p, const void *n, const void *loss_out, int32_t B, const char *who) {
    char buf[160];
    if (!x || !u || !p || !n || !loss_out) { snprintf(buf, sizeof buf, "%s: null argument", who); lgcn_set_error(buf); return 3; }
    if (B < 1 || B > x->c.max_batch) { snprintf(buf, sizeof buf, "%s: batch size out of range (1 <= B <= max_batch)", who); lgcn_set_error(buf); return 3; }
    return 0;
}

static int mf_step(lgcn_mf *x, const int32_t *users, const int32_t *pos, const int32_t *neg, int32_t B, float *loss_out, hipStream_t st) {
    const lgcn_mf_config &c = x->c;
    uint32_t *bm = c.bitmap + x->flip * x->bm_words, *stale = c.bitmap + (x->flip ^ 1) * x->bm_words;
    MfTripletArgs t{};
    t.E = c.E0; t.users = users; t.pos = pos; t.neg = neg; t.B = B; t.n_users = c.n_users; t.m_items = c.m_items;
    t.decay = c.decay; t.Bf = (float)B; t.G64 = (long long *)c.G64; t.bitmap = bm; t.terms = c.terms; t.err = c.err;
    x->step += 1;
    const double bc1 = 1.0 - pow(c.beta1, (double)x->step), bc2 = 1.0 - pow(c.beta2, (double)x->step);
    MfAdamArgs a{};
    a.P = c.E0; a.M = c.adam_m; a.V = c.adam_v; a.G64 = (long long *)c.G64; a.bitmap = bm; a.stale_bitmap = stale; a.bitmap_words = x->bm_words;
    a.n_vec = x->N * (c.d / 4); a.terms = c.terms; a.loss_out = loss_out; a.B = B; a.decay = c.decay;
    a.step_size = (float)(c.lr / bc1); a.bc2_sqrt = (float)sqrt(bc2);
    a.w1 = (float)(1.0 - c.beta1); a.beta2 = (float)c.beta2; a.omb2 = (float)(1.0 - c.beta2); a.eps = (float)c.eps;
    int64_t blocks = (a.n_vec + 255) / 256;
    if (blocks > MF_ADAM_BLOCKS_MAX) blocks = MF_ADAM_BLOCKS_MAX;
    DISPATCH_D(c.d, {
        constexpr int TPB = 256 / (D / 4);
        hipLaunchKernelGGL((k_mf_triplet<D>), dim3((unsigned)(((int64_t)B + TPB - 1) / TPB)), dim3(256), 0, st, t);
        hipLaunchKernelGGL((k_mf_adam<D>), dim3((unsigned)blocks + 1), dim3(256), 0, st, a);
    });
    x->flip ^= 1;
    HIP_OK(hipGetLastError());
    return 0;
}

extern "C" int lgcn_mf_train_step(lgcn_mf *mf, const int32_t *users, const int32_t *pos, const int32_t *neg, int32_t B,
                                  float *loss_out, void *stream) {
    if (int rc = mf_check_batch(mf, users, pos, neg, loss_out, B, "lgcn_mf_train_step")) return rc;
    return mf_step(mf, users, pos, neg, B, loss_out, (hipStream_t)stream);
}

extern "C" int lgcn_mf_train_epoch(lgcn_mf *mf, const int32_t *users, const int32_t *pos, const int32_t *neg, int64_t T, int32_t B,
                                   float *loss_out, void *stream) {
    if (int rc = mf_check_batch(mf, users, pos, neg, loss_out, B, "lgcn_mf_train_epoch")) return rc;
    int64_t i = 0;
    for (int64_t t = 0; t < T; t += B, i++) {
        const int32_t b = (int32_t)((T - t) < B ? (T - t) : B);
        if (int rc = mf_step(mf, users + t, pos + t, neg + t, b, loss_out + 3 * i, (hipStream_t)stream)) return rc;
    }
    return 0;
}

extern "C" int lgcn_mf_check(lgcn_mf *mf, void *stream) {
    if (!mf) { lgcn_set_error("lgcn_mf_check: null context"); return 3; }
    int32_t flag = 0;
    HIP_OK(hipMemcpyAsync(&flag, mf->c.err, sizeof flag, hipMemcpyDeviceToHost, (hipStream_t)stream));
    HIP_OK(hipStreamSynchronize((hipStream_t)stream));
    if (flag) {
        HIP_OK(hipMemsetAsync(mf->c.err, 0, sizeof flag, (hipStream_t)stream));
        lgcn_set_error("device flagged an out-of-range user/item id in a batch");
    }
    return flag;
}
```

graph-and-sequential-recommendation-systems_amd/csrc/lgcn_train.cpp:

```cpp
#include <math.h>
#include <stdint.h>
#include <stdio.h>
#include <stdlib.h>
#include <string.h>
#include <algorithm>
#include <new>
#include <vector>

#include "lgcn_internal.h"

struct lgcn_ctx {
    lgcn_train_config c;
    int64_t step;
    int64_t N;
    int64_t bm_words;
    int flip;
    void *act[LGCN_MAX_LAYERS + 1];
    int fwd_layers;
    float *g32;
    bf16_t *e0b;
    void *e0q;
    bool e0b_fresh;
    bool in_loop;
    lgcn_graph *hub_graph;
    int32_t hub_nnz;
    int64_t hub_rows;
    bool dp_local;
    int dp_rank;
    bool variant;
    float *tvar;
    uint32_t *item_bitmap;
    long long *gate_partials;
    long long *gate_total;
    int32_t gate_P, gate_wgs;
    int32_t *cnt;
    float *colsum;
    float drop_keep; uint64_t drop_seed; DropArgs dr;
    int32_t lw_n; float lw[LGCN_MAX_LAYERS + 1];
    bool fold_g32;
    uint16_t *mult; int64_t mult_cap;
    const uint16_t *fold_mult;
    int32_t *arrive;
    int64_t folded_steps;
    struct SlotForm { const int32_t *negs; int64_t stride; int32_t R; bool on; } mn;
    int32_t loss_kind; float loss_temp;
    void *ib_ws; int32_t ib_cap;
    int32_t ib_score; const float *ib_logq;
    int32_t ib_mix;
    int32_t store_policy, wt_adam, wt_fwd;
    int32_t hn_m; uint64_t hn_seed; int32_t *hn_sel, *hn_out;
    float au_gamma; void *au_ws; int32_t au_cap;
};
#ifndef LGCN_STORE_POLICY_DEFAULT
#define LGCN_STORE_POLICY_DEFAULT LGCN_STORE_ADAM
#endif
static int store_policy_initial() {
    const char *e = getenv("LGCN_STORE_POLICY");
    if (!e) return LGCN_STORE_POLICY_DEFAULT;
    if (e[0] < '0' || e[0] > '0' + (LGCN_STORE_ADAM | LGCN_STORE_XLAST) || e[1] != '\0') return -1;
    return e[0] - '0';
}
int64_t lgcn_fold_segment_steps() {
    const char *e = getenv("LGCN_FOLD_SEGMENT");
    const long v = e ? atol(e) : 0;
    return v > 0 ? (int64_t)v : 1024;
}
struct LoopScope {
    lgcn_ctx *x;
    explicit LoopScope(lgcn_ctx *x_) : x(x_) { x->in_loop = true; x->e0b_fresh = false; }
    ~LoopScope() { x->in_loop = false; x->e0b_fresh = false; }
};
struct SlotScope {
    lgcn_ctx *x;
    SlotScope(lgcn_ctx *x_, const int32_t *negs, int64_t stride, int32_t R) : x(x_) { x->mn = {negs, stride, R, true}; }
    ~SlotScope() { x->mn = {}; }
};

extern "C" int lgcn_ctx_create(const lgcn_train_config *cfg, lgcn_ctx **out) {
    if (!cfg || !out) { lgcn_set_error("lgcn_ctx_create: null argument"); return 3; }
    const lgcn_train_config &c = *cfg;
    if (!c.graph || !c.E0 || !c.adam_m || !c.adam_v || !c.G64 ||
        !c.bitmap || !c.terms || !c.err) { lgcn_set_error("lgcn_ctx_create: null buffer"); return 3; }
    if (c.K < 1 || c.K > LGCN_MAX_LAYERS) { lgcn_set_error("lgcn_ctx_create: K out of range"); return 3; }
    if ((c.K > 1 || c.dense_last) && !c.act) { lgcn_set_error("lgcn_ctx_create: activation workspace missing"); return 3; }
    if (c.d != 32 && c.d != 64 && c.d != 128 && c.d != 256) { lgcn_set_error("embedding dim must be 32, 64, 128 or 256"); return 3; }
    if (check_dtype(c.act_dtype)) return 3;
    if (c.act_dtype == LGCN_FP8 && c.d < 64) { lgcn_set_error("lgcn_ctx_create: fp8 activation storage needs an embedding dim of 64, 128 or 256"); return 3; }
    if (c.act_dtype == LGCN_FP8 && (c.item_pop || c.i2i)) { lgcn_set_error("lgcn_ctx_create: fp8 activation storage is implemented for the default model, not with the optional branches"); return 3; }
    if (c.n_users <= 0 || c.n_users >= c.graph->n_rows || c.max_batch <= 0) { lgcn_set_error("lgcn_ctx_create: bad sizes"); return 3; }
    if (c.d > c.graph->d_max) { lgcn_set_error("lgcn_ctx_create: d exceeds the graph's d_max"); return 3; }
    const bool gate = c.item_pop != nullptr, smooth = c.i2i != nullptr;
    if (gate || smooth) {
        if (!c.dense_last) { lgcn_set_error("lgcn_ctx_create: the optional branches need dense_last = 1 (every layer propagated densely)"); return 3; }
        const int64_t m_items = c.graph->n_rows - c.n_users;
        if (smooth && (!c.i2i_t || c.i2i->n_rows != m_items || c.i2i_t->n_rows != m_items || c.i2i->d_max < c.d || c.i2i_t->d_max < c.d)) {
            lgcn_set_error("lgcn_ctx_create: i2i / i2i_t must be [m_items, m_items] graphs with d_max >= d"); return 3; }
        if (gate && (!c.gate_params || !c.gate_adam_m || !c.gate_adam_v || !c.gate_grad || c.pop_hidden < 1 || c.pop_hidden > GATE_HMAX ||
                     c.gate_hidden < 1 || c.gate_hidden > GATE_HMAX || c.d > 128 || !(c.pop_gate_temp > 0.f))) {
            lgcn_set_error("lgcn_ctx_create: popularity gate needs its parameter / Adam buffers, hidden sizes in 1..64, d <= 128, temperature > 0"); return 3; }
    }
    if (c.reg_ego && (gate || smooth)) { lgcn_set_error("lgcn_ctx_create: reg_ego (upstream's L2 term) is defined for the default model only, not with the optional branches"); return 3; }
    const int policy = store_policy_initial();
    if (policy < 0) { lgcn_set_error("lgcn_ctx_create: LGCN_STORE_POLICY must be one of 0, 1, 2, 3 (LGCN_STORE_* bits)"); return 3; }
    lgcn_ctx *x = new (std::nothrow) lgcn_ctx;
    if (!x) { lgcn_set_error("out of memory"); return 4; }
    x->store_policy = policy; x->wt_adam = 0; x->wt_fwd = 0;
    x->c = c; x->step = 0; x->N = c.graph->n_rows; x->cnt = nullptr; x->colsum = nullptr;
    x->drop_keep = 1.f; x->drop_seed = 0; x->dr = DropArgs{};
    x->lw_n = 0; for (int k = 0; k <= LGCN_MAX_LAYERS; k++) x->lw[k] = 0.f;
    x->fold_g32 = true; x->mult = nullptr; x->mult_cap = 0; x->fold_mult = nullptr; x->arrive = nullptr; x->folded_steps = 0;
    x->mn = {};
    x->loss_kind = LGCN_LOSS_BPR; x->loss_temp = 1.f; x->ib_ws = nullptr; x->ib_cap = 0;
    x->ib_score = LGCN_SCORE_DOT; x->ib_logq = nullptr; x->ib_mix = 0;
    x->hn_m = 0; x->hn_seed = 0; x->hn_sel = nullptr; x->hn_out = nullptr;
    x->au_gamma = 0.f; x->au_ws = nullptr; x->au_cap = 0;
    x->bm_words = (x->N + 31) / 32; x->flip = 0;
    const size_t stride = table_bytes(x->N, c.d, c.act_dtype);
    for (int k = 0; k <= LGCN_MAX_LAYERS; k++) x->act[k] = nullptr;
    x->fwd_layers = c.dense_last ? c.K : c.K - 1;
    for (int k = 1; k <= x->fwd_layers; k++) x->act[k] = (char *)c.act + (size_t)(k - 1) * stride;
    x->g32 = nullptr; x->e0b = nullptr; x->e0q = nullptr; x->e0b_fresh = false; x->in_loop = false; x->dp_local = false; x->dp_rank = -1;
    x->hub_graph = nullptr; x->hub_nnz = 0; x->hub_rows = 0;
    x->variant = gate || smooth; x->tvar = nullptr; x->item_bitmap = nullptr; x->gate_partials = nullptr; x->gate_total = nullptr; x->gate_P = 0; x->gate_wgs = 0;
    const size_t gbytes = (size_t)x->N * c.d * sizeof(float);
    bool ok = hipMalloc((void **)&x->g32, gbytes) == hipSuccess && hipMemset(x->g32, 0, gbytes) == hipSuccess;
    if (ok) ok = hipMalloc((void **)&x->colsum, sizeof(float) * 3 * (size_t)c.max_batch) == hipSuccess;
    if (ok && c.reg_ego) ok = hipMalloc((void **)&x->cnt, sizeof(int32_t) * (size_t)x->N) == hipSuccess && hipMemset(x->cnt, 0, sizeof(int32_t) * (size_t)x->N) == hipSuccess;
    if (ok && x->variant) ok = hipMalloc((void **)&x->tvar, gbytes) == hipSuccess;
    if (ok && smooth) {
        const size_t wb = sizeof(uint32_t) * (size_t)((x->N - c.n_users + 31) / 32);
        ok = hipMalloc((void **)&x->item_bitmap, wb) == hipSuccess && hipMemset(x->item_bitmap, 0, wb) == hipSuccess;
    }
    if (ok && gate) {
        x->gate_P = 2 * c.pop_hidden + c.d * c.pop_hidden + c.d + 2 * c.d * c.gate_hidden + 2 * c.gate_hidden + 1;
        x->gate_wgs = (c.max_batch + GATE_TPB - 1) / GATE_TPB;
        ok = hipMalloc((void **)&x->gate_partials, sizeof(long long) * ((size_t)x->gate_wgs + 1) * x->gate_P) == hipSuccess;
        if (ok) x->gate_total = x->gate_partials + (size_t)x->gate_wgs * x->gate_P;
    }
    if (ok && c.act_dtype == LGCN_BF16 && c.K >= 2) ok = hipMalloc((void **)&x->e0b, gbytes / 2) == hipSuccess;
    if (ok && c.act_dtype == LGCN_FP8 && c.K >= 2) ok = hipMalloc(&x->e0q, table_bytes(x->N, c.d, LGCN_FP8)) == hipSuccess;
    if (ok && !c.dense_last) {
        const int32_t thr = c.hub_nnz == 0 ? TRIPLET_HUB_NNZ : c.hub_nnz;
        if (thr > 0) {
            std::vector<int32_t> ip((size_t)x->N + 1), hubs;
            ok = hipMemcpy(ip.data(), c.graph->indptr, sizeof(int32_t) * ip.size(), hipMemcpyDeviceToHost) == hipSuccess;
            for (int64_t r = 0; ok && r < x->N; r++) if (ip[(size_t)r + 1] - ip[(size_t)r] > thr) hubs.push_back((int32_t)r);
            if (ok && !hubs.empty()) {
                int32_t *dh = nullptr;
                ok = hipMalloc((void **)&dh, sizeof(int32_t) * hubs.size()) == hipSuccess &&
                     hipMemcpy(dh, hubs.data(), sizeof(int32_t) * hubs.size(), hipMemcpyHostToDevice) == hipSuccess;
                const int32_t hub_chunk = c.hub_chunk > 0 ? c.hub_chunk : TRIPLET_HUB_CHUNK;
                if (ok) ok = lgcn_graph_create_impl(c.graph->indptr, c.graph->indices, c.graph->vals, x->N, c.graph->nnz, c.d, dh,
                                               (int64_t)hubs.size(), nullptr, hub_chunk, &x->hub_graph) == 0;
                if (dh) (void)hipFree(dh);
                x->hub_nnz = thr; x->hub_rows = (int64_t)hubs.size();
            }
        }
    }
    if (!ok) {
        if (x->g32) (void)hipFree(x->g32);
        if (x->colsum) (void)hipFree(x->colsum);
        if (x->cnt) (void)hipFree(x->cnt);
        if (x->arrive) (void)hipFree(x->arrive);
        if (x->tvar) (void)hipFree(x->tvar);
        if (x->item_bitmap) (void)hipFree(x->item_bitmap);
        if (x->gate_partials) (void)hipFree(x->gate_partials);
        if (x->e0b) (void)hipFree(x->e0b);
        if (x->e0q) (void)hipFree(x->e0q);
        if (x->hub_graph) lgcn_graph_destroy(x->hub_graph);
        delete x;
        lgcn_set_error("lgcn_ctx_create: cannot allocate the library-owned tables (N*d*4 bytes fp32 gradient rows, N*d*2 bf16 parameters)");
        return 4;
    }
    *out = x;
    return 0;
}
extern "C" void lgcn_ctx_destroy(lgcn_ctx *ctx) {
    if (!ctx) return;
    if (ctx->g32) (void)hipFree(ctx->g32);
    if (ctx->colsum) (void)hipFree(ctx->colsum);
    if (ctx->cnt) (void)hipFree(ctx->cnt);
    if (ctx->arrive) (void)hipFree(ctx->arrive);
    if (ctx->mult) (void)hipFree(ctx->mult);
    if (ctx->ib_ws) (void)hipFree(ctx->ib_ws);
    if (ctx->hn_sel) (void)hipFree(ctx->hn_sel);
    if (ctx->au_ws) (void)hipFree(ctx->au_ws);
    if (ctx->tvar) (void)hipFree(ctx->tvar);
    if (ctx->item_bitmap) (void)hipFree(ctx->item_bitmap);
    if (ctx->gate_partials) (void)hipFree(ctx->gate_partials);
    if (ctx->e0b) (void)hipFree(ctx->e0b);
    if (ctx->e0q) (void)hipFree(ctx->e0q);
    if (ctx->hub_graph) lgcn_graph_destroy(ctx->hub_graph);
    delete ctx;
}
extern "C" int lgcn_ctx_set_dp_local(lgcn_ctx *ctx, int on) {
    if (!ctx) { lgcn_set_error("lgcn_ctx_set_dp_local: null context"); return 3; }
    ctx->dp_local = on != 0; ctx->dp_rank = -1;
    return 0;
}
extern "C" int lgcn_ctx_set_fold_g32(lgcn_ctx *ctx, int on) {
    if (!ctx) { lgcn_set_error("lgcn_ctx_set_fold_g32: null context"); return 3; }
    ctx->fold_g32 = on != 0;
    return 0;
}
extern "C" int64_t lgcn_ctx_folded_steps(const lgcn_ctx *ctx) { return ctx ? ctx->folded_steps : -1; }
extern "C" int lgcn_ctx_set_store_policy(lgcn_ctx *ctx, int bits) {
    if (bits & ~(LGCN_STORE_ADAM | LGCN_STORE_XLAST)) { lgcn_set_error("lgcn_ctx_set_store_policy: unknown store policy bits (LGCN_STORE_ADAM | LGCN_STORE_XLAST)"); return 3; }
    if (!ctx) { lgcn_set_error("lgcn_ctx_set_store_policy: null context"); return 3; }
    ctx->store_policy = bits;
    return 0;
}
extern "C" int lgcn_ctx_get_store_policy(const lgcn_ctx *ctx, int32_t *launch_out) {
    if (launch_out) { launch_out[0] = ctx ? ctx->wt_adam : 0; launch_out[1] = ctx ? ctx->wt_fwd : 0; }
    return ctx ? ctx->store_policy : store_policy_initial();
}
extern "C" int lgcn_ctx_copy_arrivals(const lgcn_ctx *ctx, int32_t *dst_host, int64_t n) {
    if (!ctx || !dst_host) { lgcn_set_error("lgcn_ctx_copy_arrivals: null argument"); return 3; }
    if (ctx->variant || n < 0 || n > ctx->N) { lgcn_set_error("lgcn_ctx_copy_arrivals: the context has no arrival array of that size"); return 3; }
    if (!ctx->arrive) { memset(dst_host, 0, sizeof(int32_t) * (size_t)n); return 0; }
    HIP_OK(hipDeviceSynchronize());
    HIP_OK(hipMemcpy(dst_host, ctx->arrive, sizeof(int32_t) * (size_t)n, hipMemcpyDeviceToHost));
    return 0;
}
extern "C" int64_t lgcn_ctx_get_step(const lgcn_ctx *ctx) { return ctx ? ctx->step : -1; }
extern "C" int64_t lgcn_ctx_hub_rows(const lgcn_ctx *ctx) { return (ctx && ctx->hub_graph) ? ctx->hub_rows : 0; }
extern "C" void lgcn_ctx_set_step(lgcn_ctx *ctx, int64_t s) { if (ctx) ctx->step = s; }
extern "C" void lgcn_ctx_set_lr(lgcn_ctx *ctx, double lr) { if (ctx) ctx->c.lr = lr; }
extern "C" int lgcn_ctx_set_dropout(lgcn_ctx *ctx, float keep_prob, uint64_t seed) {
    if (!ctx) { lgcn_set_error("lgcn_ctx_set_dropout: null context"); return 3; }
    if (!drop_prob_ok(keep_prob)) { lgcn_set_error("lgcn_ctx_set_dropout: dropout keep_prob must be in (0, 1]"); return 3; }
    if (ctx->c.act_dtype == LGCN_FP8) { lgcn_set_error("lgcn_ctx_set_dropout: edge dropout is not implemented for LGCN_FP8 activation storage"); return 3; }
    if (ctx->variant) { lgcn_set_error("lgcn_ctx_set_dropout: edge dropout is not implemented with the optional branches (item-item smoothing / popularity gate)"); return 3; }
    if (ctx->lw_n && keep_prob < 1.f) { lgcn_set_error("lgcn_ctx_set_dropout: edge dropout is not implemented together with layer weights (lgcn_ctx_set_layer_weights)"); return 3; }
    ctx->drop_keep = keep_prob; ctx->drop_seed = seed; ctx->dr = DropArgs{};
    return 0;
}
static int refuse_dropout(const lgcn_ctx *x, const char *who) {
    if (!x || !(x->drop_keep < 1.f)) return 0;
    char buf[192];
    snprintf(buf, sizeof buf, "%s: edge dropout (lgcn_ctx_set_dropout) is implemented for the single-GPU step only", who);
    lgcn_set_error(buf);
    return 3;
}

extern "C" int lgcn_ctx_set_layer_weights(lgcn_ctx *ctx, const float *w_host, int32_t n) {
    if (!ctx) { lgcn_set_error("lgcn_ctx_set_layer_weights: null context"); return 3; }
    if (!w_host || n == 0) { ctx->lw_n = 0; return 0; }
    if (n < 0 || n > LGCN_MAX_LAYERS + 1) n = -1;
    if (int rc = lgcn_check_layer_weights("lgcn_ctx_set_layer_weights", w_host, n, ctx->c.K)) return rc;
    if (ctx->c.act_dtype == LGCN_FP8) { lgcn_set_error("lgcn_ctx_set_layer_weights: layer weights are not implemented for LGCN_FP8 activation storage"); return 3; }
    if (ctx->variant) { lgcn_set_error("lgcn_ctx_set_layer_weights: layer weights are not implemented with the optional branches (item-item smoothing / popularity gate)"); return 3; }
    if (ctx->drop_keep < 1.f) { lgcn_set_error("lgcn_ctx_set_layer_weights: layer weights are not implemented together with edge dropout (lgcn_ctx_set_dropout)"); return 3; }
    for (int k = 0; k < n; k++) ctx->lw[k] = w_host[k];
    ctx->lw_n = n;
    return 0;
}
extern "C" int32_t lgcn_ctx_get_layer_weights(const lgcn_ctx *ctx, float *w_out) {
    if (!ctx || !ctx->lw_n) return 0;
    if (w_out) for (int k = 0; k < ctx->lw_n; k++) w_out[k] = ctx->lw[k];
    return ctx->lw_n;
}
static int refuse_layer_weights(const lgcn_ctx *x, const char *who) {
    if (!x || !x->lw_n) return 0;
    char buf[192];
    snprintf(buf, sizeof buf, "%s: layer weights (lgcn_ctx_set_layer_weights) are implemented for the single-GPU step only", who);
    lgcn_set_error(buf);
    return 3;
}

struct InBatchWs {
    size_t U, P, sbb, uid, pid, mrg, part, invu, invp, lq, words, icap;
    InBatchWs(int32_t cap_, int d, int32_t R_max) {
        const size_t cap = (size_t)cap_;
        const size_t parts = (size_t)(R_max ? lgcn_inbatch_mix_parts(cap_, R_max) : lgcn_inbatch_parts(cap_));
        size_t at = 0;
        auto take = [&at](size_t n) { const size_t o = at; at += n; return o; };
        icap = (size_t)(1 + R_max) * cap;
        U = take(cap * d); P = take(icap * d); sbb = take(cap); uid = take(cap); pid = take(icap); mrg = take(2 * cap);
        part = take(2 * cap * parts); invu = take(cap); invp = take(icap); lq = take(icap);
        words = at;
        if (R_max) words = std::max(words, InBatchWs(cap_, d, 0).words);
    }
};

static int refuse_loss_config(const lgcn_ctx *ctx, float temperature, const char *what, const char *slots) {
    char buf[256];
    const char *fmt = nullptr;
    if (!(temperature > 0.f) || !isfinite(temperature)) fmt = "lgcn_ctx_set_loss: %s needs a finite temperature > 0";
    else if (ctx->c.act_dtype == LGCN_FP8) fmt = "lgcn_ctx_set_loss: %s is not implemented for LGCN_FP8 activation storage";
    else if (ctx->variant) fmt = "lgcn_ctx_set_loss: %s is not implemented with the optional branches (item-item smoothing / popularity gate)";
    else if (!ctx->c.dense_last) fmt = "lgcn_ctx_set_loss: %s needs a context with dense_last = 1 (the gathered last layer has no %s slot form)";
    if (!fmt) return 0;
    snprintf(buf, sizeof buf, fmt, what, slots);
    lgcn_set_error(buf);
    return 3;
}

extern "C" int lgcn_ctx_set_loss(lgcn_ctx *ctx, int32_t kind, float temperature) {
// ... 266 lines not shown
        g.inv_B = 1.0f / (float)B_global; g.lam = c.decay / (float)B_global;
        g.G64 = atomics ? (long long *)c.G64 : nullptr; g.bitmap = bm; g.item_bitmap = c.i2i ? x->item_bitmap : nullptr;
        g.stale_bitmap = stale; g.bitmap_words = x->bm_words; g.terms = c.terms + (exchange ? 0 : b_off); g.terms_stride = B_global; g.err = c.err;
        g.contrib = c.contrib; g.shard = shard; g.exchange = exchange ? 1 : 0;
        if (int rc = lgcn_gate_launch(g, c.d, st)) return rc;
        if (exchange)
            lgcn_gate_rank_total_launch((const long long *)x->gate_partials, (int32_t)((B_local + GATE_TPB - 1) / GATE_TPB), x->gate_P,
                                        (long long *)(c.contrib + tail), st);
    } else {
        BprArgs a{};
        a.X0 = x->tvar; a.K = 0; a.dense_last = 1;
        a.n_users = c.n_users; a.N = x->N; a.users = users + b_off; a.pos = pos + b_off; a.neg = neg + b_off; a.B_local = B_local; a.shard = shard;
        a.inv_B = 1.0f / (float)B_global; a.lam = c.decay / (float)B_global;
        a.G64 = atomics ? (long long *)c.G64 : nullptr; a.bitmap = bm; a.stale_bitmap = stale; a.bitmap_words = x->bm_words;
        a.item_bitmap = x->item_bitmap; a.terms = c.terms; a.err = c.err; a.terms_off = exchange ? 0 : b_off; a.terms_stride = B_global;
        a.contrib = c.contrib; a.exchange = exchange ? 1 : 0;
        return lgcn_triplet_launch(a, c.d, LGCN_F32, false, false, st);
    }
    return 0;
}

static SlotArgs slot_args(const lgcn_ctx *x, const int32_t *users, const int32_t *pos, const int32_t *neg, int32_t B,
                          const float *gathered, int32_t shard, int32_t world, float *loss_out) {
    const lgcn_train_config &c = x->c;
    SlotArgs s{};
    s.users = users; s.pos = pos; s.neg = neg; s.B = B; s.n_users = c.n_users; s.N = x->N;
    s.G64 = (long long *)c.G64; s.G32 = x->g32; s.div = x->lw_n ? 1.f : (float)(c.K + 1);
    s.bitmap = c.bitmap + x->flip * x->bm_words; s.gathered = gathered; s.shard = shard; s.world = world;
    s.terms = c.terms; s.loss_out = loss_out; s.decay = c.decay; s.skip_rank = -1;
    s.ent_coeff = c.item_pop ? c.gate_entropy_coeff : 0.f;
    s.blk = gathered ? dp_block_floats(x, shard) : 0;
    s.item_bitmap = (x->variant && c.i2i) ? x->item_bitmap : nullptr;
    s.cnt = x->cnt;
    return s;
}
static SlotArgsMulti slot_args_multi(const lgcn_ctx *x, const int32_t *users, const int32_t *pos, int32_t B, float *loss_out) {
    SlotArgsMulti m{};
    m.s = slot_args(x, users, pos, nullptr, B, nullptr, B, 1, loss_out);
    m.negs = x->mn.negs; m.neg_stride = x->mn.stride; m.R = x->mn.R;
    return m;
}
static void *bwd_buffer(const lgcn_ctx *x, int k) {
    return (x->c.K == 2) ? x->act[1] : x->act[1 + ((x->c.K - k) & 1)];
}

static int backward_layer(lgcn_ctx *x, int k, const int32_t *users, const int32_t *pos, const int32_t *neg, int32_t B,
                          const float *gathered, int32_t shard, float *loss_out, bool fused_finish, hipStream_t st) {
    const lgcn_train_config &c = x->c;
    const bool first = (k == c.K), last = (k == 1);
    if (first) {
        if (x->mn.on) {
            SlotArgsMulti s = slot_args_multi(x, users, pos, B, loss_out);
            if (int rc = lgcn_g32_multi_launch(s, c.d, st)) return rc;
        } else if (!x->fold_mult) {
            SlotArgs s = slot_args(x, users, pos, neg, B, gathered, shard, 1, loss_out);
            if (int rc = lgcn_g32_launch(s, c.d, st)) return rc;
        }
        if (x->variant && c.i2i) {
            { int rc0 = graph_acquire(c.i2i_t, st); if (rc0) return rc0; }
            const int64_t ioff = (int64_t)c.n_users * c.d, m_items = x->N - c.n_users;
            SpmmArgs h = graph_spmm(c.i2i_t);
            h.G32 = x->g32 + ioff; h.bitmap = x->item_bitmap; h.Y = x->tvar + ioff; h.div = (float)(c.K + 1); h.remap = c.xcd_remap;
            int rc = lgcn_spmm_launch(h, M_SPARSE | M_ADDG, c.d, LGCN_F32, LGCN_F32, st);
            if (rc) return rc;
            HIP_OK(hipMemcpyAsync(x->g32 + ioff, x->tvar + ioff, sizeof(float) * (size_t)m_items * c.d, hipMemcpyDeviceToDevice, st));
            lgcn_flag_range_launch(c.bitmap + x->flip * x->bm_words, (int64_t)c.n_users, x->N, st);
        }
    }
    SpmmArgs a = base_spmm(x);
    a.dr = x->dr; a.dr.tr = 1;
    a.X = first ? nullptr : bwd_buffer(x, k + 1);
    if (!last) a.Y = bwd_buffer(x, k);
    else {
        const double bc1 = 1.0 - pow(c.beta1, (double)x->step);
        const double bc2 = 1.0 - pow(c.beta2, (double)x->step);
        a.P = c.E0; a.M = c.adam_m; a.V = c.adam_v;
        a.cnt = x->cnt; a.lam = c.decay / (float)B;
        if (x->mn.R > 0) a.lam = c.decay / (float)((int64_t)B * x->mn.R);
        a.Pb = (x->e0b && x->in_loop && fused_finish) ? x->e0b : nullptr;
        a.Pq = (x->e0q && x->in_loop && fused_finish) ? x->e0q : nullptr;
        x->e0b_fresh = a.Pb != nullptr || a.Pq != nullptr;
        if (x->store_policy & LGCN_STORE_ADAM) a.wt = LGCN_STORE_ARG_MV | ((a.Pb || a.Pq) ? LGCN_STORE_ARG_P : 0);
        x->wt_adam = a.wt;
        a.step_size = (float)(c.lr / bc1); a.bc2_sqrt = (float)sqrt(bc2);
        a.w1 = (float)(1.0 - c.beta1); a.beta2 = (float)c.beta2; a.omb2 = (float)(1.0 - c.beta2); a.eps = (float)c.eps;
        if (!first && fused_finish) {
            a.clear = 1; a.terms = c.terms; a.gathered = gathered; a.loss_out = loss_out;
            a.B = B; a.shard = shard; a.decay = c.decay; a.ent_coeff = c.item_pop ? c.gate_entropy_coeff : 0.f;
            a.blk = gathered ? dp_block_floats(x, shard) : 0;
        }
    }
    const int prev_dt = first ? LGCN_F32 : c.act_dtype;
    int mode = M_ADDG | (first ? M_SPARSE : 0) | (last ? M_ADAM : 0);
    if (x->lw_n) {
        a.w_in = first ? x->lw[c.K] : 1.f; a.w_add = x->lw[k - 1];
        mode |= M_WTS;
    }
    return lgcn_spmm_launch(a, mode, c.d, prev_dt, last ? LGCN_F32 : c.act_dtype, st);
}

static int run_backward(lgcn_ctx *x, const int32_t *users, const int32_t *pos, const int32_t *neg, int32_t B,
                        const float *gathered, int32_t shard, int32_t world, float *loss_out, hipStream_t st, bool gate_reduced = false) {
    const lgcn_train_config &c = x->c;
    { int rc0 = graph_acquire(c.graph, st); if (rc0) return rc0; }
    SlotArgs s = slot_args(x, users, pos, neg, B, gathered, shard, world, loss_out);
    if (gathered) {
        s.skip_rank = x->dp_local ? x->dp_rank : -1;
        if (int rc = lgcn_scatter_launch(s, c.d, st)) return rc;
    }
    x->step += 1;
    for (int k = c.K; k >= 1; k--) {
        int rc = backward_layer(x, k, users, pos, neg, B, gathered, shard, loss_out, true, st);
        if (rc) return rc;
    }
    if (x->variant && c.item_pop) {
        GateAdamArgs ga{};
        if (gathered) {
            ga.src = (const long long *)(gathered + dp_block_tail(x, shard)); ga.n_src = world; ga.stride = dp_block_floats(x, shard) / 2;
        } else if (gate_reduced) {
            ga.src = x->gate_total; ga.n_src = 1; ga.stride = x->gate_P;
        } else { ga.src = x->gate_partials; ga.n_src = (B + GATE_TPB - 1) / GATE_TPB; ga.stride = x->gate_P; }
        ga.P = x->gate_P;
        ga.params = c.gate_params; ga.m = c.gate_adam_m; ga.v = c.gate_adam_v; ga.grad_out = c.gate_grad;
        const double bc1 = 1.0 - pow(c.beta1, (double)x->step), bc2 = 1.0 - pow(c.beta2, (double)x->step);
        ga.step_size = (float)(c.lr / bc1); ga.bc2_sqrt = (float)sqrt(bc2);
        ga.w1 = (float)(1.0 - c.beta1); ga.beta2 = (float)c.beta2; ga.omb2 = (float)(1.0 - c.beta2); ga.eps = (float)c.eps;
        lgcn_gate_adam_launch(ga, st);
    }
    if (c.K >= 2) { x->flip ^= 1; return 0; }
    if (x->mn.on) {
        SlotArgsMulti sm = slot_args_multi(x, users, pos, B, loss_out);
        return lgcn_finish_multi_launch(sm, c.d, st);
    }
    if (int rc = lgcn_finish_launch(s, c.d, st)) return rc;
    if (x->variant && c.i2i) {
        HIP_OK(hipMemsetAsync(c.bitmap + x->flip * x->bm_words, 0, sizeof(uint32_t) * (size_t)x->bm_words, st));
    }
    return 0;
}

static MultiNegArgs multineg_args(const lgcn_ctx *x, const int32_t *users, const int32_t *pos, int32_t B) {
    const lgcn_train_config &c = x->c;
    MultiNegArgs a{};
    a.X0 = c.E0; a.K = c.K;
    for (int k = 1; k <= x->fwd_layers; k++) a.Xl[k] = x->act[k];
    a.n_users = c.n_users; a.N = x->N;
    a.users = users; a.pos = pos; a.negs = x->mn.negs; a.neg_stride = x->mn.stride; a.R = x->mn.R; a.B = B;
    a.lam = c.decay / (float)B;
    if (x->mn.R > 0) {
        const float BR = (float)((int64_t)B * x->mn.R);
        a.inv_BR = 1.0f / BR; a.inv_R = 1.0f / (float)x->mn.R; a.lam_n = c.decay / BR;
    }
    a.G64 = (long long *)c.G64; a.bitmap = c.bitmap + x->flip * x->bm_words;
    a.stale_bitmap = c.bitmap + (x->flip ^ 1) * x->bm_words; a.bitmap_words = x->bm_words;
    a.terms = c.terms; a.terms_stride = B; a.err = c.err;
    a.reg_ego = c.reg_ego; a.cnt = x->cnt;
    for (int k = 0; k < x->lw_n; k++) a.w[k] = x->lw[k];
    a.loss = x->loss_kind;
    if (x->loss_kind != LGCN_LOSS_BPR) {
        a.tau = x->loss_temp; a.inv_tauB = (float)(1.0 / ((double)x->loss_temp * (double)B));
    }
    return a;
}

static int run_inbatch(lgcn_ctx *x, const int32_t *users, const int32_t *pos, int32_t B, hipStream_t st) {
    const lgcn_train_config &c = x->c;
    const bool mix = x->mn.R > 0;
    const InBatchWs ws(x->ib_cap, c.d, mix ? x->ib_mix : 0);
    float *w = (float *)x->ib_ws;
    InBatchArgs ia{};
    ia.m = multineg_args(x, users, pos, B);
    ia.cap = x->ib_cap;
    ia.U = w + ws.U; ia.P = w + ws.P; ia.sbb = w + ws.sbb;
    ia.uid = (int32_t *)(w + ws.uid); ia.pid = (int32_t *)(w + ws.pid);
    ia.mrg = w + ws.mrg; ia.part = w + ws.part;
    if (mix) { ia.mix = 1; ia.icap = (int32_t)ws.icap; ia.xinvu = w + ws.invu; ia.xinvp = w + ws.invp; ia.xlq = w + ws.lq; }
    ia.score = x->ib_score; ia.item_logq = x->ib_logq;
    return lgcn_inbatch_launch(ia, c.d, c.act_dtype, x->lw_n != 0, st);
}

static int run_directau(lgcn_ctx *x, const int32_t *users, const int32_t *pos, int32_t B, hipStream_t st) {
    const lgcn_train_config &c = x->c;
    const DirectAuWs ws(x->au_cap, c.d);
    float *w = (float *)x->au_ws;
    DirectAuArgs da{};
    da.m = multineg_args(x, users, pos, B);
    da.m.tau = 0.f; da.m.inv_tauB = 0.f;
    da.cap = x->au_cap; da.gamma = x->au_gamma;
    da.X = w + ws.X; da.Y = w + ws.Y; da.invx = w + ws.invx; da.invy = w + ws.invy; da.qx = w + ws.qx; da.qy = w + ws.qy; da.al = w + ws.al;
    da.uid = (int32_t *)(w + ws.uid); da.pid = (int32_t *)(w + ws.pid); da.part = w + ws.part; da.scal = w + ws.scal;
    return lgcn_directau_launch(da, c.d, c.act_dtype, x->lw_n != 0, st);
}

static int run_step(lgcn_ctx *x, const int32_t *users, const int32_t *pos, const int32_t *neg, int32_t B, float *loss_out, hipStream_t st) {
    const lgcn_train_config &c = x->c;
    int rc;
    x->dr = make_drop(x->drop_keep, x->drop_seed, x->step, 0);
    if ((rc = run_forward(x, st))) return rc;
    if (!x->mn.on) rc = x->variant ? run_variant_loss(x, users, pos, neg, B, 0, B, B, true, false, st) : run_bpr(x, users, pos, neg, B, 0, B, B, true, false, st);
    else if (x->loss_kind == LGCN_LOSS_INBATCH) rc = run_inbatch(x, users, pos, B, st);
    else if (x->loss_kind == LGCN_LOSS_DIRECTAU) rc = run_directau(x, users, pos, B, st);
    else if (x->hn_m) {
        HardNegArgs h{};
        h.m = multineg_args(x, users, pos, B);
        h.inv_B = 1.0f / (float)B; h.top_m = x->hn_m; h.seed = x->hn_seed; h.step = x->step;
        h.sel_id = x->hn_sel; h.sel_out = x->hn_out;
        rc = lgcn_hardneg_launch(h, c.d, c.act_dtype, x->lw_n != 0, st);
        x->mn = {};
// ... 444 lines not shown
```

graph-and-sequential-recommendation-systems_amd/model.py:

```python
import ctypes as C

import numpy as np
import torch
from torch import nn
import torch.nn.functional as F

from . import world
from . import _lib


def _act_code(name):
    return {'fp32': _lib.F32, 'bf16': _lib.BF16, 'fp8': _lib.FP8}[name]


def _act_tables(n_tables, N, d, act_dtype, dev):
    if act_dtype == _lib.FP8:
        return torch.zeros(n_tables, int(_lib.load().lgcn_table_bytes(N, d, _lib.FP8)), dtype=torch.uint8, device=dev)
    return torch.zeros(n_tables, N, d, dtype=torch.float32 if act_dtype == _lib.F32 else torch.bfloat16, device=dev)


def _check_layer_weights(w, K, what):
    w = np.asarray(w, dtype=np.float64).reshape(-1)
    if w.size != K + 1:
        raise ValueError(f"{what}: {w.size} layer weights for --layer {K} (K + 1 = {K + 1} are needed)")
# ... 644 lines not shown
        if self.neg_ratio > 1 and not dense_last:
            dense_last = True
            if not self._neg_ratio_said:
                world.cprint(f"[neg_ratio] --neg_ratio {self.neg_ratio}: the last layer is propagated densely (dense_last = 1)")
                self._neg_ratio_said = True
        if self.loss_kind != 'bpr' and not dense_last:
            dense_last = True
            if not self._loss_said:
                world.cprint(f"[loss] --loss {self.loss_kind}: the last layer is propagated densely (dense_last = 1)")
                self._loss_said = True
        return dense_last

    def _ctx_workspace(self, st, max_batch, dp_world, dense_last, variants, act_dtype):
        N, d, K, dev = self.n_users + self.m_items, self.latent_dim, self.n_layers, self._table.device
        self._step_workspace(st, 3 * max_batch)
        st['act'] = _act_tables(max(1, K if dense_last else K - 1), N, d, act_dtype, dev)
        shard = (max_batch + dp_world - 1) // dp_world
        gate_p = sum(prm.numel() for prm in self.gate_parameters()) if (variants and self.use_pop_gate) else 0
        st['contrib'] = torch.zeros(3 * shard * d + 3 * shard + 2 + 2 * gate_p, dtype=torch.float32, device=dev)
        st['hard_neg_sel'] = (torch.full((max_batch,), -1, dtype=torch.int32, device=dev)
                              if self.hard_neg and int(self.config.get('hard_neg_record', 0)) else None)
        if self.inbatch_logq and (st.get('item_logq') is None or st['item_logq'].device != dev):
            st['item_logq'] = self._item_logq.to(device=dev, dtype=torch.float32).contiguous()
        if variants and self.i2i_active:
            for key, mat in (('i2i_s', self._i2i), ('i2i_ts', self._i2i.T.tocsr())):
                if key not in st:
                    mat = mat.tocsr().astype(np.float32)
                    mat.sort_indices()
                    st[key] = _lib.Graph(torch.from_numpy(mat.indptr.astype(np.int32)).to(dev), torch.from_numpy(mat.indices.astype(np.int32)).to(dev),
                                         torch.from_numpy((np.float32(self.i2i_alpha) * mat.data).astype(np.float32)).to(dev), d_max=d)
        if variants and self.use_pop_gate:
            self._pack_gate()
            P = self._gate_flat.numel()
            for key in ('gate_m', 'gate_v', 'gate_grad'):
                if key not in st or st[key].numel() != P:
                    st[key] = torch.zeros(P, dtype=torch.float32, device=dev)
            st['item_pop'] = self.item_pop_scalar.to(device=dev, dtype=torch.float32).contiguous()

    def _ctx_config(self, st, max_batch, rows, dense_last, variants, act_dtype):
        cfg = self._fill_step_config(_lib.TrainConfig(), st, max_batch)
        cfg.graph = (st['graph_rs'] if rows == 'owned' else st['graph']).handle
        cfg.K, cfg.act_dtype = self.n_layers, act_dtype
        cfg.act, cfg.contrib = st['act'].data_ptr(), st['contrib'].data_ptr()
        cfg.reg_ego = int(self._reg_ego())
        if cfg.reg_ego and variants:
            raise _lib.LgcnError("--reg_rows ego (upstream LightGCN's L2 term) is defined for the default model, not with "
                                 "--use_pop_gate / --use_item_item")
        cfg.xcd_remap = int(self.config.get('xcd_remap', 1))
        cfg.dense_last = int(dense_last)
        cfg.hub_nnz = int(self.config.get('hub_nnz', 0))
        cfg.hub_chunk = int(self.config.get('hub_chunk', 0))
        if variants and self.i2i_active:
            cfg.i2i, cfg.i2i_t = st['i2i_s'].handle, st['i2i_ts'].handle
        if variants and self.use_pop_gate:
            cfg.item_pop, cfg.gate_params = st['item_pop'].data_ptr(), self._gate_flat.data_ptr()
            cfg.gate_adam_m, cfg.gate_adam_v, cfg.gate_grad = st['gate_m'].data_ptr(), st['gate_v'].data_ptr(), st['gate_grad'].data_ptr()
            cfg.pop_hidden, cfg.gate_hidden = self.pop_hidden, self.gate_hidden
            cfg.gate_entropy_coeff, cfg.pop_gate_temp = self.gate_entropy_coeff, self.pop_gate_temp
        return cfg

    def _ctx_setters(self, st, old_step):
        out = [('lgcn_ctx_set_step', (old_step,))]
        if self.dropout:
            out.append(('lgcn_ctx_set_dropout', (self.keep_prob, int(self.config.get('seed', 2020)) & (2 ** 64 - 1))))
        if self.layer_weights is not None:
            w = np.ascontiguousarray(self.layer_weights, dtype=np.float32)
            out.append(('lgcn_ctx_set_layer_weights', (_lib.npp(w), int(w.size))))
        if self.loss_kind == 'directau':
            out.append(('lgcn_ctx_set_directau', (float(self.au_gamma),)))
        elif self.loss_kind != 'bpr':
            out.append(('lgcn_ctx_set_loss', (_lib.LOSS_INBATCH if self.loss_kind == 'inbatch' else _lib.LOSS_SOFTMAX, float(self.softmax_temp))))
        if self.score_kind != 'dot' or self.inbatch_logq:
            out.append(('lgcn_ctx_set_inbatch_scores', (_lib.SCORE_COSINE if self.score_kind == 'cosine' else _lib.SCORE_DOT,
                                                        _lib.tp(st['item_logq']) if self.inbatch_logq else None)))
        if self.inbatch_mix:
            out.append(('lgcn_ctx_set_inbatch_mix', (int(self.neg_ratio),)))
        if self.hard_neg:
            out.append(('lgcn_ctx_set_hard_neg', (int(self.hard_neg), int(self.config.get('seed', 2020)) & (2 ** 64 - 1),
                                                  _lib.tp(st['hard_neg_sel']) if st.get('hard_neg_sel') is not None else None)))
        if str(self.config.get('fold_g32', 1)).strip().lower() in ('0', 'false', 'off'):
            out.append(('lgcn_ctx_set_fold_g32', (0,)))
        if self.config.get('store_policy') is not None:
            out.append(('lgcn_ctx_set_store_policy', (int(self.config['store_policy']),)))
        return out

    def _dense_last(self, batch):
        mode = str(self.config.get('dense_last', 'auto'))
        if mode in ('0', '1'):
            return mode == '1'
        deg = np.diff(self._adj.indptr).astype(np.float64)
        du, di = deg[:self.n_users], deg[self.n_users:]
        per_triplet = du.mean() + (di * di).sum() / max(di.sum(), 1.0) + di.mean()
        return bool(batch * per_triplet > 0.3 * self._adj.nnz)

    def _spmm(self, x):
        return self._state()['graph'].spmm(x.float(), _lib.F32)

    @property
    def i2i_active(self):
        return self.use_item_item and self._i2i is not None and self.i2i_alpha > 0.0

    @property
    def has_variants(self):
        return self.use_pop_gate or self.i2i_active

    def _i2i_apply(self, x, transpose):
        st = self._state()
        key = 'i2i_t' if transpose else 'i2i'
        if key not in st:
            m = self._i2i.T.tocsr() if transpose else self._i2i
            m.sort_indices()
            dev = self._table.device
            st[key] = _lib.Graph(torch.from_numpy(m.indptr.astype(np.int32)).to(dev), torch.from_numpy(m.indices.astype(np.int32)).to(dev),
                                 torch.from_numpy(m.data.astype(np.float32)).to(dev), d_max=self.latent_dim)
        x = x.contiguous().float()
        return x + self.i2i_alpha * st[key].spmm(x, _lib.F32)

    def _fuse_item_embeddings(self, items_emb):
        pop_vec = self.pop_mlp(self.item_pop_scalar.unsqueeze(1))
        gate_logit = self.gate_mlp(torch.cat([items_emb, pop_vec], dim=1))
        if self.pop_gate_temp != 1.0:
            gate_logit = gate_logit / self.pop_gate_temp
        gate = torch.sigmoid(gate_logit)
        self._last_item_gate = gate
        return gate * items_emb + (1.0 - gate) * pop_vec

    def _propagate_dense(self):
        st = self._state()
        N, d, K = self.n_users + self.m_items, self.latent_dim, self.n_layers
        act_dtype = _act_code(self._act())
        work = st.get('eval_work')
        if K > 1 and (work is None or st.get('eval_work_dtype') != act_dtype):
            work = st['eval_work'] = _act_tables(K - 1, N, d, act_dtype, self._table.device)
            st['eval_work_dtype'] = act_dtype
        out = torch.empty(N, d, dtype=torch.float32, device=self._table.device)
        if self.layer_weights is not None:
            w = np.ascontiguousarray(self.layer_weights, dtype=np.float32)
            _lib.check(_lib.load().lgcn_propagate_weighted(
                st['graph'].handle, _lib.tp(self._table), K, d, act_dtype, _lib.tp(work) if K > 1 else None,
                w.ctypes.data_as(C.c_void_p), _lib.tp(out), _lib.current_stream()), "lgcn_propagate_weighted")
            return out
        _lib.check(_lib.load().lgcn_propagate_mean(
            st['graph'].handle, _lib.tp(self._table), K, d, act_dtype, _lib.tp(work) if K > 1 else None,
            _lib.tp(out), _lib.current_stream()), "lgcn_propagate_mean")
        return out

    def invalidate_cache(self):
        self._cache = None
        self._rating_cache = None
        self._cosine_cache = None

    def train(self, mode=True):
        self.invalidate_cache()
        return super().train(mode)

    def propagated_table(self):
        if self._cache is None:
            with torch.no_grad():
                out = self._propagate_dense()
                cr = getattr(self, 'col_range', None)
                if cr is not None and cr[1] - cr[0] < cr[2]:
                    import torch.distributed as dist
                    if not (dist.is_available() and dist.is_initialized() and dist.get_world_size() * (cr[1] - cr[0]) == cr[2]):
                        raise _lib.LgcnError("this model holds columns %d..%d of %d: evaluation needs the process group that holds the others" % cr)
                    parts = [torch.empty_like(out) for _ in range(dist.get_world_size())]
                    dist.all_gather(parts, out.contiguous())
# ... 222 lines not shown
            if not self.inbatch_mix:
                return ("lgcn_train_step_inbatch", (u, p, T), T, held) if step else ("lgcn_train_epoch_inbatch", (u, p, T, batch_size), T, held)
            negs = self._negs_rn(neg, T, dev, mixed=True)
            n, R, held = _lib.tp(negs), int(negs.shape[0]), (users, pos, negs)
            return ("lgcn_train_step_inbatch_mix", (u, p, n, T, R, T), T, held) if step else ("lgcn_train_epoch_inbatch_mix", (u, p, n, R, T, batch_size), T, held)
        if self.loss_kind == 'softmax' and self._neg_dim(neg) == 1:
            neg = self._ids(neg, dev).reshape(1, -1)
        if self._neg_dim(neg) == 2:
            users, pos = self._ids(users, dev), self._ids(pos, dev)
            T = int(users.numel())
            negs = self._negs_rn(neg, T, dev)
            if negs is not None:
                u, p, n, R, held = _lib.tp(users), _lib.tp(pos), _lib.tp(negs), int(negs.shape[0]), (users, pos, negs)
                return ("lgcn_train_step_multi", (u, p, n, T, R, T), T, held) if step else ("lgcn_train_epoch_multi", (u, p, n, R, T, batch_size), T, held)
            neg = self._ids(neg, dev).reshape(-1)
        if not (step and all(torch.is_tensor(t) and t.dtype == torch.int64 and t.device == dev and t.is_contiguous() for t in (users, pos, neg))):
            return _TableModel._dispatch(self, users, pos, neg, batch_size)
        B = int(users.numel())
        ids = (_lib.tp(users), _lib.tp(pos), _lib.tp(neg), B)

        def with_scratch(st):
            if st.get('ids32') is None or st['ids32'].numel() < 3 * B:
                st['ids32'] = torch.empty(3 * max(B, st['max_batch']), dtype=torch.int32, device=dev)
            return (*ids, _lib.tp(st['ids32']))
        return "lgcn_train_step_i64", with_scratch, B, (users, pos, neg)


class PureMF(_TableModel):
    has_variants = False
    fused_variants = False
    use_pop_gate = False
    dropout = False
    layer_weights = None
    _CTX = {'destroy': 'lgcn_mf_destroy', 'get_step': 'lgcn_mf_get_step', 'set_step': 'lgcn_mf_set_step', 'set_lr': 'lgcn_mf_set_lr',
            'check': 'lgcn_mf_check', 'step': 'lgcn_mf_train_step', 'epoch': 'lgcn_mf_train_epoch'}

    def __init__(self, config, dataset):
        super().__init__(config, dataset)
        no = "is not implemented for --model mf"
        if config.get('use_pop_gate', False):
            raise _lib.LgcnError(f"--use_pop_gate {no} (the popularity gate belongs to LightGCN)")
        if config.get('use_item_item', False):
            raise _lib.LgcnError(f"--use_item_item {no} (the item-item smoothing belongs to LightGCN)")
        if int(config.get('dropout', 0)):
            raise _lib.LgcnError(f"--dropout 1 {no} (there is no graph whose edges could be dropped)")
        lw = config.get('layer_weights', 'mean')
        if not (lw is None or (isinstance(lw, str) and lw.strip().lower() == 'mean')):
            raise _lib.LgcnError(f"--layer_weights {lw} {no} (there are no layers to combine)")
        if config.get('use_ppr_weights', False):
            raise _lib.LgcnError(f"--use_ppr_weights {no} (there are no layers to combine)")
        if self._act() != 'fp32':
            raise _lib.LgcnError(f"--act_dtype {config.get('act_dtype')} {no} (fp32 tables only)")
        if int(config.get('hard_neg', 0)) != 0:
            raise _lib.LgcnError(f"--hard_neg {config.get('hard_neg')} {no} (hard negatives are picked among LightGCN's --neg_ratio candidates)")
        if int(config.get('neg_ratio', 1)) != 1:
            raise _lib.LgcnError(f"--neg_ratio {config.get('neg_ratio')} {no} (the matrix-factorisation step trains on triplets, "
                                 "one negative per positive)")
        if str(config.get('loss', 'bpr')).strip().lower() != 'bpr':
            raise _lib.LgcnError(f"--loss {config.get('loss')} {no} (the matrix-factorisation step computes the BPR loss)")
        if str(config.get('score', 'dot')).strip().lower() != 'dot':
            raise _lib.LgcnError(f"--score {config.get('score')} {no} (an option of LightGCN's --loss inbatch)")
        if str(config.get('inbatch_logq', 0)).strip().lower() not in ('0', 'false'):
            raise _lib.LgcnError(f"--inbatch_logq {config.get('inbatch_logq')} {no} (an option of LightGCN's --loss inbatch)")
        if str(config.get('inbatch_mix', 0)).strip().lower() not in ('0', 'false'):
            raise _lib.LgcnError(f"--inbatch_mix {config.get('inbatch_mix')} {no} (an option of LightGCN's --loss inbatch)")
        if self.latent_dim not in (32, 64, 128, 256):
            raise ValueError("latent_dim_rec must be 32, 64, 128 or 256 for the HIP kernels")
        if self.n_users + self.m_items >= 2 ** 31:
            raise ValueError("n_users + m_items must stay below 2^31")
        self.embedding_user = nn.Embedding(self.n_users, self.latent_dim)
        self.embedding_item = nn.Embedding(self.m_items, self.latent_dim)
        self._bind_table()
        self.f = nn.Sigmoid()

    def _ctx_stale(self, st, dp_world, rows):
        return st.get('table_ptr') != self._table.data_ptr()

    def _make_ctx(self, max_batch, dp_world=1, rows=None):
        st = self._dev
        old_step = self._retire_ctx(st)
        self._step_workspace(st, 2 * max_batch)
        cfg = self._fill_step_config(_lib.MfConfig(), st, max_batch)
        cfg.m_items = self.m_items
        st['ctx'] = self._create_ctx('lgcn_mf_create', cfg, [('lgcn_mf_set_step', (old_step,))])
        st['max_batch'], st['table_ptr'] = max_batch, self._table.data_ptr()

    def propagated_table(self):
        return self._table

    def rating_table(self):
        return self._table

    def computer(self):
        return self.embedding_user.weight, self.embedding_item.weight

    def getUsersRating(self, users):
        all_users, all_items = self.computer()
        return self.f(torch.matmul(all_users[users.long()], all_items.t()))

    def getEmbedding(self, users, pos_items, neg_items):
        all_users, all_items = self.computer()
        return all_users[users.long()], all_items[pos_items.long()], all_items[neg_items.long()], all_users, all_items

    def bpr_loss(self, users, pos, neg):
        u, pos_e, neg_e, _, _ = self.getEmbedding(users, pos, neg)
        pos_scores = torch.sum(u * pos_e, dim=1)
        neg_scores = torch.sum(u * neg_e, dim=1)
        loss = torch.mean(F.softplus(neg_scores - pos_scores))
        reg_loss = (0.5 * (u.norm(2).pow(2) + pos_e.norm(2).pow(2) + neg_e.norm(2).pow(2))) / float(u.shape[0])
        return loss, reg_loss

    def forward(self, users, items):
        all_users, all_items = self.computer()
        return self.f(torch.sum(all_users[users.long()] * all_items[items.long()], dim=1))
```

include/lgcn_hip.h:

```cpp
#ifndef LGCN_HIP_H
#define LGCN_HIP_H

#include <stdint.h>

#ifdef __cplusplus
extern "C" {
#endif

#define LGCN_ABI_VERSION 13
#define LGCN_MAX_LAYERS 8

enum { LGCN_F32 = 0, LGCN_BF16 = 1, LGCN_FP8 = 2 };
int64_t lgcn_table_bytes(int64_t n_rows, int32_t d, int32_t dtype);
int lgcn_to_fp8(const float *src, void *dst, int64_t n_rows, int32_t d, void *stream);

int lgcn_abi_version(void);
const char *lgcn_last_error(void);
int lgcn_device_available(void);

void lgcn_sampling_seed(unsigned int seed);
int lgcn_sampling_randint(int end);
int lgcn_sample_negative(int user_num, int item_num, int64_t train_num,
                         const int64_t *indptr, const int32_t *indices,
                         int neg_num, int32_t *S_out);
// ... 84 lines not shown
    const float *item_pop;
    float *gate_params;
    float *gate_adam_m;
    float *gate_adam_v;
    float *gate_grad;
    int32_t pop_hidden;
    int32_t gate_hidden;
    float gate_entropy_coeff;
    float pop_gate_temp;
    int32_t reg_ego;
} lgcn_train_config;

int lgcn_ctx_create(const lgcn_train_config *cfg, lgcn_ctx **out);
void lgcn_ctx_destroy(lgcn_ctx *ctx);
int64_t lgcn_ctx_get_step(const lgcn_ctx *ctx);
int64_t lgcn_ctx_hub_rows(const lgcn_ctx *ctx);
void lgcn_ctx_set_step(lgcn_ctx *ctx, int64_t step);
void lgcn_ctx_set_lr(lgcn_ctx *ctx, double lr);
int lgcn_ctx_set_dropout(lgcn_ctx *ctx, float keep_prob, uint64_t seed);
int lgcn_ctx_set_layer_weights(lgcn_ctx *ctx, const float *w_host, int32_t n);
int32_t lgcn_ctx_get_layer_weights(const lgcn_ctx *ctx, float *w_out);
int lgcn_ctx_set_dp_local(lgcn_ctx *ctx, int on);

int lgcn_train_step(lgcn_ctx *ctx, const int32_t *users, const int32_t *pos, const int32_t *neg,
                    int32_t B, float *loss_out, void *stream);

int lgcn_train_step_i64(lgcn_ctx *ctx, const int64_t *users, const int64_t *pos, const int64_t *neg,
                        int32_t B, int32_t *ids_scratch, float *loss_out, void *stream);

int lgcn_train_epoch(lgcn_ctx *ctx, const int32_t *users, const int32_t *pos, const int32_t *neg,
                     int64_t T, int32_t B, float *loss_out, void *stream);

#define LGCN_MAX_NEG_RATIO 16
int lgcn_train_step_multi(lgcn_ctx *ctx, const int32_t *users, const int32_t *pos,
                          const int32_t *negs, int64_t neg_stride, int32_t R,
                          int32_t B, float *loss_out, void *stream);
int lgcn_train_epoch_multi(lgcn_ctx *ctx, const int32_t *users, const int32_t *pos,
                           const int32_t *negs , int32_t R,
                           int64_t T, int32_t B, float *loss_out, void *stream);
#define LGCN_LOSS_BPR 0
#define LGCN_LOSS_SOFTMAX 1
int lgcn_ctx_set_loss(lgcn_ctx *ctx, int32_t kind, float temperature);
int32_t lgcn_ctx_get_loss(const lgcn_ctx *ctx, float *temperature_out);

#define LGCN_LOSS_INBATCH 2
int lgcn_train_step_inbatch(lgcn_ctx *ctx, const int32_t *users, const int32_t *pos, int32_t B, float *loss_out, void *stream);
int lgcn_train_epoch_inbatch(lgcn_ctx *ctx, const int32_t *users, const int32_t *pos, int64_t T, int32_t B, float *loss_out,
                             void *stream);

#define LGCN_SCORE_DOT 0
#define LGCN_SCORE_COSINE 1
int lgcn_ctx_set_inbatch_scores(lgcn_ctx *ctx, int score, const float *item_logq);
int lgcn_ctx_get_inbatch_scores(const lgcn_ctx *ctx, const float **item_logq);

int lgcn_ctx_set_inbatch_mix(lgcn_ctx *ctx, int32_t R_max);
int32_t lgcn_ctx_get_inbatch_mix(const lgcn_ctx *ctx);
int lgcn_train_step_inbatch_mix(lgcn_ctx *ctx, const int32_t *users, const int32_t *pos, const int32_t *negs, int64_t neg_stride,
                                int32_t R, int32_t B, float *loss_out, void *stream);
int lgcn_train_epoch_inbatch_mix(lgcn_ctx *ctx, const int32_t *users, const int32_t *pos, const int32_t *negs, int32_t R,
                                 int64_t T, int32_t B, float *loss_out, void *stream);

#define LGCN_LOSS_DIRECTAU 4
int lgcn_ctx_set_directau(lgcn_ctx *ctx, float gamma);
int lgcn_ctx_get_directau(const lgcn_ctx *ctx, float *gamma);
int lgcn_train_step_directau(lgcn_ctx *ctx, const int32_t *users, const int32_t *pos, int32_t B, float *loss_out, void *stream);
int lgcn_train_epoch_directau(lgcn_ctx *ctx, const int32_t *users, const int32_t *pos, int64_t T, int32_t B, float *loss_out,
                              void *stream);

int lgcn_ctx_set_hard_neg(lgcn_ctx *ctx, int32_t top_m, uint64_t seed, int32_t *sel_out);
int32_t lgcn_ctx_get_hard_neg(const lgcn_ctx *ctx);
uint32_t lgcn_hard_neg_rank(uint64_t seed, int64_t step, int32_t b, int32_t M);

int lgcn_ctx_set_fold_g32(lgcn_ctx *ctx, int on);
int64_t lgcn_ctx_folded_steps(const lgcn_ctx *ctx);
int lgcn_ctx_copy_arrivals(const lgcn_ctx *ctx, int32_t *dst_host, int64_t n);

#define LGCN_STORE_ADAM 1
#define LGCN_STORE_XLAST 2
int lgcn_ctx_set_store_policy(lgcn_ctx *ctx, int bits);
#define LGCN_STORE_ARG_MV 1
#define LGCN_STORE_ARG_P 2
#define LGCN_STORE_ARG_Y 4
int lgcn_ctx_get_store_policy(const lgcn_ctx *ctx, int32_t *launch_out);
int lgcn_slot_multiplicity(const int32_t *users, const int32_t *pos, const int32_t *neg, int64_t T, int32_t B,
                           int32_t n_users, int64_t N, uint16_t *mult_out, void *stream);

int64_t lgcn_dp_block_floats(const lgcn_ctx *ctx, int32_t B_global, int32_t world);
int lgcn_train_step_dp_part1(lgcn_ctx *ctx, const int32_t *users, const int32_t *pos,
                             const int32_t *neg, int32_t B_global, int32_t world, int32_t rank,
                             void *stream);
int lgcn_train_step_dp_dense_part1(lgcn_ctx *ctx, const int32_t *users, const int32_t *pos,
                                   const int32_t *neg, int32_t B_global, int32_t world, int32_t rank,
                                   void *stream);
int lgcn_ctx_gate_total(const lgcn_ctx *ctx, void **buf, int32_t *count);
int lgcn_train_step_dp_part2(lgcn_ctx *ctx, const int32_t *users, const int32_t *pos,
                             const int32_t *neg, int32_t B_global, int32_t world,
                             const float *gathered, float *loss_out, void *stream);

int lgcn_train_step_cols_part1(lgcn_ctx *ctx, const int32_t *users, const int32_t *pos, const int32_t *neg,
                               int32_t B, float **partials, void *stream);
int lgcn_train_step_cols_part2(lgcn_ctx *ctx, const int32_t *users, const int32_t *pos, const int32_t *neg,
                               int32_t B, float *loss_out, void *stream);

int lgcn_eval_topk(const float *E, int32_t n_users, int32_t m_items, int32_t d,
                   const int32_t *users, int32_t n_eval,
                   const int64_t *train_indptr, const int32_t *train_indices,
                   int32_t K, int32_t *topk_items, float *topk_scores, void *stream);
int64_t lgcn_eval_mask_words(int32_t m_items, int32_t n_eval);
int lgcn_eval_build_masks(const int32_t *users, int32_t n_eval, const int64_t *train_indptr, const int32_t *train_indices,
                          int32_t m_items, uint32_t *masks, void *stream);
int lgcn_eval_topk_masked(const float *E, int32_t n_users, int32_t m_items, int32_t d,
                          const int32_t *users, int32_t n_eval,
                          const int64_t *train_indptr, const int32_t *train_indices,
                          int32_t K, int32_t *topk_items, float *topk_scores, const uint32_t *masks, void *stream);
int lgcn_eval_topk_fp32(const float *E, int32_t n_users, int32_t m_items, int32_t d,
                        const int32_t *users, int32_t n_eval,
                        const int64_t *train_indptr, const int32_t *train_indices,
                        int32_t K, int32_t *topk_items, float *topk_scores, void *stream);
int lgcn_eval_metrics(const int32_t *topk_items, int32_t n_eval, int32_t K,
                      const int64_t *test_indptr, const int32_t *test_items_sorted,
                      const int32_t *ks, int32_t n_ks, double *per_user, double *sums, void *stream);
#define LGCN_EVAL_FP32 1
int32_t lgcn_eval_kmax(void);
int lgcn_eval_topk_ex(const float *E, int32_t n_users, int32_t m_items, int32_t d,
                      const int32_t *users, int32_t n_eval,
                      const int64_t *train_indptr, const int32_t *train_indices, const uint32_t *masks,
                      int32_t K, int32_t *topk_items, float *topk_scores, int64_t out_capacity,
                      int32_t flags, void *stream);
int lgcn_eval_metrics_ex(const int32_t *topk_items, int32_t n_eval, int32_t K,
                         const int64_t *test_indptr, const int32_t *test_items_sorted,
                         const int32_t *ks, int32_t n_ks, double *per_user, double *sums, void *stream);
int lgcn_eval_ranks(const float *E, int32_t n_users, int32_t m_items, int32_t d,
                    const int32_t *users, int32_t n_eval,
                    const int64_t *train_indptr, const int32_t *train_indices,
                    const int64_t *test_indptr, const int32_t *test_items_sorted, int64_t n_test,
                    float *test_scores, int32_t *gt, int32_t *eq, int32_t flags, void *stream);
int lgcn_eval_rank_metrics(int32_t n_eval, int32_t m_items, const int32_t *users,
                           const int64_t *train_indptr, const int32_t *train_indices,
                           const int64_t *test_indptr, const int32_t *test_items_sorted, int64_t n_test,
                           const float *test_scores, const int32_t *gt, const int32_t *eq,
                           const int32_t *ks, int32_t n_ks, double *per_user, double *sums, void *stream);

enum { LGCN_I2I_COOC = 0, LGCN_I2I_JACCARD = 1, LGCN_I2I_PMI = 2 };
int lgcn_i2i_topk(const int64_t *indptr, const int32_t *indices, int64_t n_baskets, int64_t nnz, int32_t m_items,
                  int32_t topk, int32_t weight, int32_t min_basket, int32_t *cols, float *w, int32_t *len, void *stream);
int lgcn_i2i_finish(const int32_t *cols, const float *w, const int32_t *len, int32_t m_items, int32_t topk, int64_t capacity,
                    int32_t *indptr, int32_t *indices, float *vals, int64_t *nnz_out, void *stream);

#define LGCN_DP_ID_BYTES 128
enum { LGCN_DP_ROWS = 0, LGCN_DP_DENSE = 1, LGCN_DP_ROW_SHARDED = 2, LGCN_DP_COLS = 3 };
typedef struct lgcn_dp lgcn_dp;
int lgcn_dp_available(void);
int lgcn_dp_unique_id(void *id128);
int lgcn_dp_init(const void *id128, int world, int rank, lgcn_dp **out);
int lgcn_dp_init_loopback(int world, lgcn_dp **out);
void lgcn_dp_destroy(lgcn_dp *dp);
int lgcn_dp_allreduce_sum_f32(lgcn_dp *dp, float *buf, int64_t n, void *stream);
int lgcn_dp_world(const lgcn_dp *dp);
int lgcn_dp_rank(const lgcn_dp *dp);
int lgcn_train_epoch_dp(lgcn_ctx *ctx, lgcn_dp *dp, const int32_t *users, const int32_t *pos,
                        const int32_t *neg, int64_t T, int32_t B_global, int32_t reduce,
                        const int64_t *row_ranges, float *gathered, float *loss_out, void *stream);

enum { LGCN_RS_FWD = 0, LGCN_RS_BPR = 1, LGCN_RS_SCATTER = 2, LGCN_RS_BWD = 3, LGCN_RS_FINISH = 4 };
int lgcn_rs_phase(lgcn_ctx *ctx, int32_t phase, int32_t k, const int32_t *users, const int32_t *pos,
                  const int32_t *neg, int32_t B_global, int32_t world, int32_t rank,
                  const float *gathered, float *loss_out, void *stream);
int lgcn_rs_buffer(const lgcn_ctx *ctx, int32_t phase, int32_t k, void **buf, int32_t *dtype);

int lgcn_ctx_check(lgcn_ctx *ctx, void *stream);

typedef struct lgcn_mf lgcn_mf;

typedef struct {
    int32_t n_users;
    int32_t m_items;
    int32_t d;
    float *E0;
    float *adam_m;
    float *adam_v;
    int64_t *G64;
    uint32_t *bitmap;
    float *terms;
    int32_t *err;
    int32_t max_batch;
    float decay;
    double lr, beta1, beta2, eps;
} lgcn_mf_config;

int lgcn_mf_create(const lgcn_mf_config *cfg, lgcn_mf **out);
void lgcn_mf_destroy(lgcn_mf *mf);
int64_t lgcn_mf_get_step(const lgcn_mf *mf);
void lgcn_mf_set_step(lgcn_mf *mf, int64_t step);
void lgcn_mf_set_lr(lgcn_mf *mf, double lr);

int lgcn_mf_train_step(lgcn_mf *mf, const int32_t *users, const int32_t *pos, const int32_t *neg,
                       int32_t B, float *loss_out, void *stream);

int lgcn_mf_train_epoch(lgcn_mf *mf, const int32_t *users, const int32_t *pos, const int32_t *neg,
                        int64_t T, int32_t B, float *loss_out, void *stream);

int lgcn_mf_check(lgcn_mf *mf, void *stream);

#ifdef __cplusplus
}
#endif
#endif
```

Measured before the change: 8871 steps/s.

## Spread Adam epilogue across all lanes and add bit-exact short sqrt/div path

The sparse Adam epilogue in the SpMM kernel now spreads each row's elements across the full wavefront (W elements per lane), both for single-chunk rows and for rows finished by the last-arriving chunk, instead of only LPR lanes doing C elements each. This is meant to cut the serial per-lane Adam arithmetic and memory traffic per row. Separately, it adds an optional bit-exact fast path for the Adam denominator, using a hardware sqrt with correction and reciprocal-multiply division with Newton fixups, selected by LGCN_ADAM_MATH (default off), plus a probe kernel that checks exactness. The spread path is enabled by default but adds more VecF widths and store variants, and it drops the fp8/Y stores for narrow C.

```diff
diff --git a/graph-and-sequential-recommendation-systems_amd/_lib.py b/graph-and-sequential-recommendation-systems_amd/_lib.py
--- a/graph-and-sequential-recommendation-systems_amd/_lib.py
+++ b/graph-and-sequential-recommendation-systems_amd/_lib.py
@@ -171,8 +171,14 @@
     "lgcn_slot_multiplicity": (C.c_int, [_vp, _vp, _vp, C.c_int64, C.c_int32, C.c_int32, C.c_int64, _vp, _vp]),
     "lgcn_ctx_set_store_policy": (C.c_int, [_vp, C.c_int]),
     "lgcn_ctx_get_store_policy": (C.c_int, [_vp, _c_i32p]),
+    "lgcn_ctx_set_adam_math": (C.c_int, [_vp, C.c_int]),
+    "lgcn_ctx_get_adam_math": (C.c_int, [_vp]),
+    "lgcn_mf_set_adam_math": (C.c_int, [_vp, C.c_int]),
+    "lgcn_ctx_copy_shadow": (C.c_int, [_vp, _vp, C.c_int64]),
+    "lgcn_adam_denom_probe": (C.c_int, [C.c_int, C.c_int, _vp, C.c_int32, C.c_float, C.c_uint32, C.c_uint64, _vp, _vp]),
 }
 
+ADAM_MATH_SHORT = 1
 STORE_ADAM, STORE_XLAST = 1, 2
 STORE_ARG_MV, STORE_ARG_P, STORE_ARG_Y = 1, 2, 4
 
diff --git a/graph-and-sequential-recommendation-systems_amd/csrc/lgcn_device.hip b/graph-and-sequential-recommendation-systems_amd/csrc/lgcn_device.hip
--- a/graph-and-sequential-recommendation-systems_amd/csrc/lgcn_device.hip
+++ b/graph-and-sequential-recommendation-systems_amd/csrc/lgcn_device.hip
@@ -18,6 +18,8 @@
 __device__ __forceinline__ float *fp8_scales(void *tab, int64_t n_rows, int D) { return (float *)((char *)tab + n_rows * D); }
 
 template <int C> struct VecF;
+template <> struct VecF<1> { typedef __attribute__((ext_vector_type(1))) float T; typedef __attribute__((ext_vector_type(1))) __bf16 B; };
+template <> struct VecF<2> { typedef __attribute__((ext_vector_type(2))) float T; typedef __attribute__((ext_vector_type(2))) __bf16 B; };
 template <> struct VecF<4> { typedef f32x4 T; typedef bf16x4 B; };
 template <> struct VecF<8> { typedef f32x8 T; typedef bf16x8 B; };
 template <> struct VecF<16> { typedef f32x16 T; typedef bf16x16 B; };
@@ -49,9 +51,13 @@
     asm volatile("global_store_dwordx4 %0, %1, off offset:%2 sc1\n\ts_nop 1" : : "v"(p), "v"(v), "n"(OFF) : "memory");
 }
 template <int C> __device__ __forceinline__ void storev_wt(float *p, typename VecF<C>::T v) {
-    store16_wt<0>(p, f32x4{v[0], v[1], v[2], v[3]});
-    if constexpr (C >= 8) store16_wt<16>(p, f32x4{v[4], v[5], v[6], v[7]});
-    if constexpr (C == 16) { store16_wt<32>(p, f32x4{v[8], v[9], v[10], v[11]}); store16_wt<48>(p, f32x4{v[12], v[13], v[14], v[15]}); }
+    if constexpr (C == 1) asm volatile("global_store_dword %0, %1, off sc1" : : "v"(p), "v"(v[0]) : "memory");
+    else if constexpr (C == 2) asm volatile("global_store_dwordx2 %0, %1, off sc1" : : "v"(p), "v"(v) : "memory");
+    else {
+        store16_wt<0>(p, f32x4{v[0], v[1], v[2], v[3]});
+        if constexpr (C >= 8) store16_wt<16>(p, f32x4{v[4], v[5], v[6], v[7]});
+        if constexpr (C == 16) { store16_wt<32>(p, f32x4{v[8], v[9], v[10], v[11]}); store16_wt<48>(p, f32x4{v[12], v[13], v[14], v[15]}); }
+    }
 }
 __device__ __forceinline__ void storev_wt(bf16_t *p, f32x8 v) {
     union { bf16x8 b; f32x4 f; } u; u.b = __builtin_convertvector(v, bf16x8);
@@ -340,6 +346,8 @@
                     i64x2 *q = reinterpret_cast<i64x2 *>(a.G64 + row * D + (j * (D / 16) + l) * 4);
                     q[0] = i64x2{0, 0}; q[1] = i64x2{0, 0};
                 }
+            } else if constexpr (C == 1) {
+                a.G64[off] = 0;
             } else {
                 i64x2 *q = reinterpret_cast<i64x2 *>(a.G64 + off);
 #pragma unroll
@@ -359,16 +367,26 @@
         m = m + a.w1 * (acc - m);
         v = v * a.beta2 + (a.omb2 * acc) * acc;
         V denom;
-#pragma unroll
-        for (int i = 0; i < C; i++) denom[i] = sqrtf(v[i]) / a.bc2_sqrt + a.eps;
+        constexpr bool PLAIN = D == 32 && (MODE & (M_SPARSE | M_WTS)) == (M_SPARSE | M_WTS);
+        if constexpr (PLAIN) {
+#pragma unroll
+            for (int i = 0; i < C; i++) denom[i] = sqrtf(v[i]) / a.bc2_sqrt + a.eps;
+        } else {
+            float vs[C], ds[C];
+#pragma unroll
+            for (int i = 0; i < C; i++) vs[i] = v[i];
+            adam_denom<C>(vs, ds, a.bc2_sqrt, a.rbc2, a.eps);
+#pragma unroll
+            for (int i = 0; i < C; i++) denom[i] = ds[i];
+        }
         p = p - a.step_size * (m / denom);
         row_store<D, C, IL>(a.P, row, l, p, (a.wt & LGCN_STORE_ARG_P) != 0);
         row_store<D, C, IL>(a.M, row, l, m, (a.wt & LGCN_STORE_ARG_MV) != 0); row_store<D, C, IL>(a.V, row, l, v, (a.wt & LGCN_STORE_ARG_MV) != 0);
         if constexpr (!(MODE & M_SPARSE)) {
             if (a.Pb) storev<C>(a.Pb + off, p);
-            if (a.Pq) store_row_fp8<D, C, IL>(a.Pq, a.n_rows, row, l, p);
-        }
-    } else {
+            if constexpr (C >= 4) { if (a.Pq) store_row_fp8<D, C, IL>(a.Pq, a.n_rows, row, l, p); }
+        }
+    } else if constexpr (C >= 4) {
         RowStore<D, C, TO, IL>::put(a.Y, a.n_rows, row, l, acc, (a.wt & LGCN_STORE_ARG_Y) != 0);
     }
 }
@@ -464,6 +482,9 @@
 #endif
 #ifndef SPMM_ADAM_SPLIT
 #define SPMM_ADAM_SPLIT 1
+#endif
+#ifndef SPMM_ADAM_LONG_SPREAD
+#define SPMM_ADAM_LONG_SPREAD 1
 #endif
 #ifndef SPMM_ADAM_PREFETCH_BF16
 #define SPMM_ADAM_PREFETCH_BF16 0
@@ -546,7 +567,23 @@
         const bool rflag = (MODE & M_ADDG) ? bit_set(a.bitmap, (int)row) : false;
 #endif
         Acc acc = row_gather<D, TI, SP, BIG, DROP>(PackedSrc{a.pk}, ch.y, ch.z, src, lane, stage_lds[wid], (int)row);
+        constexpr int W = D >= 64 ? D / 64 : 1;
+        constexpr bool SPREAD = SPMM_ADAM_LONG_SPREAD && (MODE & M_ADAM) != 0 && !IL && W < C;
         if (nch == 1) {
+            if constexpr (SPREAD) {
+                constexpr int SUB = C / W;
+                const int g = lane / LPR, l = lane % LPR;
+                if (64 / LPR > SUB && g >= SUB) return;
+                typename VecF<W>::T h;
+#pragma unroll
+                for (int i = 0; i < W; i++) h[i] = acc[i];
+#pragma unroll
+                for (int s = 1; s < SUB; s++) {
+#pragma unroll
+                    for (int i = 0; i < W; i++) h[i] = g == s ? acc[s * W + i] : h[i];
+                }
+                spmm_epilogue<D, TO, MODE, W, false>(a, row, l * SUB + g, h, rflag);
+            } else
             if (lane < LPR) spmm_epilogue<D, TO, MODE, C, IL>(a, row, lane, acc, rflag);
             return;
         }
@@ -565,6 +602,24 @@
         __builtin_amdgcn_fence(__ATOMIC_ACQUIRE, "agent");
         asm volatile("s_waitcnt vmcnt(0)" ::: "memory");
         if (lane == 0) __hip_atomic_store(a.lp.counters + o, 0, __ATOMIC_RELAXED, __HIP_MEMORY_SCOPE_AGENT);
+        if constexpr (SPREAD) {
+            if (D < 64 && lane >= D) return;
+            const int first = c - ch.w;
+            typedef __attribute__((address_space(1))) unsigned gu32;
+            typename VecF<W>::T tot = zerov<W>();
+            for (int k = 0; k < nch; k++) {
+                const float *src_ = a.lp.partials + (int64_t)(first + k) * D + lane * W;
+                union { typename VecF<W>::T v; unsigned long long q[W >= 2 ? W / 2 : 1]; unsigned u; } pk;
+                if constexpr (W == 1) pk.u = __hip_atomic_load((gu32 *)src_, __ATOMIC_RELAXED, __HIP_MEMORY_SCOPE_AGENT);
+                else {
+#pragma unroll
+                    for (int i = 0; i < W / 2; i++) pk.q[i] = __hip_atomic_load((gu64 *)src_ + i, __ATOMIC_RELAXED, __HIP_MEMORY_SCOPE_AGENT);
+                }
+                if (k == 0) tot = pk.v; else tot += pk.v;
+            }
+            spmm_epilogue<D, TO, MODE, W, false>(a, row, lane, tot, rflag);
+            return;
+        }
         if (lane >= LPR) return;
         const int first = c - ch.w;
         Acc tot = zerov<C>();
@@ -1377,11 +1432,61 @@
     const float g = (float)((double)q * FIXED_INV);
     a.grad_out[i] = g;
     float m = a.m[i], v = a.v[i], p = a.params[i];
-    m = m + a.w1 * (g - m);
-    v = v * a.beta2 + (a.omb2 * g) * g;
-    const float denom = sqrtf(v) / a.bc2_sqrt + a.eps;
-    p = p - a.step_size * (m / denom);
+    {
+#pragma clang fp contract(off)
+        m = m + a.w1 * (g - m);
+        v = __builtin_fmaf(a.omb2 * g, g, v * a.beta2);
+        float denom;
+        adam_denom<1>(&v, &denom, a.bc2_sqrt, a.rbc2, a.eps);
+        p = __builtin_fmaf(-a.step_size, m / denom, p);
+    }
     a.params[i] = p; a.m[i] = m; a.v[i] = v;
+}
+
+struct AdamProbeArgs { const float *c; float eps; int32_t what, adam_math; uint32_t x_first; uint64_t n_x; unsigned long long *out; };
+__global__ void __launch_bounds__(256) k_adam_denom_probe(AdamProbeArgs a) {
+    const float c = a.c[blockIdx.y], rc = (a.what == 1 || (a.adam_math & LGCN_ADAM_MATH_SHORT)) ? 1.0f / c : 0.f;
+    unsigned long long n_bad = 0, first = ~0ull;
+    for (uint64_t i = (uint64_t)blockIdx.x * 256 + threadIdx.x; i < a.n_x; i += (uint64_t)gridDim.x * 256) {
+        const uint32_t xb = a.x_first + (uint32_t)i;
+        const float x = __uint_as_float(xb);
+        float got, want;
+        if (a.what == 0) { adam_denom<1>(&x, &got, c, rc, a.eps); want = sqrtf(x) / c + a.eps; }
+        else { got = adam_div_const(x, c, rc); want = x / c; }
+        if (__float_as_uint(got) != __float_as_uint(want)) {
+            n_bad++;
+            const unsigned long long id = ((unsigned long long)blockIdx.y << 32) | xb;
+            first = id < first ? id : first;
+        }
+    }
+    if (n_bad) { atomicAdd(a.out, n_bad); atomicMin(a.out + 1, first); }
+}
+extern "C" int lgcn_adam_denom_probe(int what, int adam_math, const float *c, int32_t n_c, float eps, uint32_t x_first, uint64_t n_x,
+                                     uint64_t *out_host, void *stream) {
+    if (!c || !out_host) { lgcn_set_error("lgcn_adam_denom_probe: null argument"); return 3; }
+    if (what < 0 || what > 1 || (adam_math & ~LGCN_ADAM_MATH_SHORT)) { lgcn_set_error("lgcn_adam_denom_probe: unknown `what` or adam_math bits"); return 3; }
+    if (n_c < 1 || n_c > 65535 || n_x < 1 || n_x > (1ull << 32)) { lgcn_set_error("lgcn_adam_denom_probe: n_c must be 1..65535 and n_x 1..2^32"); return 3; }
+    hipStream_t st = (hipStream_t)stream;
+    char *buf = nullptr;
+    const size_t cb = sizeof(float) * (size_t)n_c, off = (cb + 15) / 16 * 16;
+    HIP_OK(hipMalloc((void **)&buf, off + 16));
+    unsigned long long init[2] = {0ull, ~0ull};
+    AdamProbeArgs a{};
+    a.c = (const float *)buf; a.eps = eps; a.what = what; a.adam_math = adam_math; a.x_first = x_first; a.n_x = n_x;
+    a.out = (unsigned long long *)(buf + off);
+    int rc = 0;
+    if (hipMemcpyAsync(buf, c, cb, hipMemcpyHostToDevice, st) != hipSuccess ||
+        hipMemcpyAsync(buf + off, init, sizeof init, hipMemcpyHostToDevice, st) != hipSuccess) rc = 1;
+    if (!rc) {
+        const uint64_t want = (n_x + 255) / 256;
+        hipLaunchKernelGGL(k_adam_denom_probe, dim3((unsigned)(want < 2048 ? want : 2048), (unsigned)n_c), dim3(256), 0, st, a);
+        if (hipGetLastError() != hipSuccess || hipMemcpyAsync(init, buf + off, sizeof init, hipMemcpyDeviceToHost, st) != hipSuccess ||
+            hipStreamSynchronize(st) != hipSuccess) rc = 1;
+    }
+    (void)hipFree(buf);
+    if (rc) { lgcn_set_error("lgcn_adam_denom_probe: a HIP call failed"); return 1; }
+    out_host[0] = init[0]; out_host[1] = init[1];
+    return 0;
 }
 __global__ void __launch_bounds__(256) k_gate_rank_total(const long long *partials, int32_t n_part, int32_t P, long long *out) {
     const int i = blockIdx.x * 256 + threadIdx.x;
diff --git a/graph-and-sequential-recommendation-systems_amd/csrc/lgcn_device_common.h b/graph-and-sequential-recommendation-systems_amd/csrc/lgcn_device_common.h
--- a/graph-and-sequential-recommendation-systems_amd/csrc/lgcn_device_common.h
+++ b/graph-and-sequential-recommendation-systems_amd/csrc/lgcn_device_common.h
@@ -65,6 +65,42 @@
     }
 }
 
+__device__ __forceinline__ float adam_sqrt_core(float x) {
+#pragma clang fp contract(off)
+    float s = __builtin_amdgcn_sqrtf(x);
+    const float dn = __int_as_float(__float_as_int(s) - 1), up = __int_as_float(__float_as_int(s) + 1);
+    const float rd = __builtin_fmaf(-dn, s, x), ru = __builtin_fmaf(-up, s, x);
+    s = rd <= 0.f ? dn : s;
+    s = ru > 0.f ? up : s;
+    return s;
+}
+__device__ __forceinline__ float adam_div_const(float x, float c, float rc) {
+#pragma clang fp contract(off)
+    float q = x * rc;
+    float r = __builtin_fmaf(-c, q, x);
+    q = __builtin_fmaf(r, rc, q);
+    r = __builtin_fmaf(-c, q, x);
+    q = __builtin_fmaf(r, rc, q);
+    return q;
+}
+template <int C> __device__ __forceinline__ bool adam_denom_short(const float *v, float rc) {
+    uint32_t lo = __float_as_uint(v[0]), hi = lo;
+#pragma unroll
+    for (int i = 1; i < C; i++) { const uint32_t u = __float_as_uint(v[i]); lo = min(lo, u); hi = max(hi, u); }
+    const bool bad = lo < 0x0F800000u  || hi >= 0x7F800000u  || rc == 0.f;
+    return __ballot(bad) == 0ull;
+}
+template <int C> __device__ __forceinline__ void adam_denom(const float *v, float *denom, float c, float rc, float eps) {
+#pragma clang fp contract(off)
+    if (adam_denom_short<C>(v, rc)) {
+#pragma unroll
+        for (int i = 0; i < C; i++) denom[i] = adam_div_const(adam_sqrt_core(v[i]), c, rc) + eps;
+    } else {
+#pragma unroll
+        for (int i = 0; i < C; i++) denom[i] = sqrtf(v[i]) / c + eps;
+    }
+}
+
 __device__ __forceinline__ void fixed_add(long long *g64, float g) {
     atomicAdd((unsigned long long *)g64, (unsigned long long)__double2ll_rn((double)g * FIXED_SCALE));
 }
diff --git a/graph-and-sequential-recommendation-systems_amd/csrc/lgcn_kernels.h b/graph-and-sequential-recommendation-systems_amd/csrc/lgcn_kernels.h
--- a/graph-and-sequential-recommendation-systems_amd/csrc/lgcn_kernels.h
+++ b/graph-and-sequential-recommendation-systems_amd/csrc/lgcn_kernels.h
@@ -52,12 +52,16 @@
     int64_t blk;
     float step_size, bc2_sqrt, w1, beta2, omb2, eps;
     int remap;
+    float rbc2;
     const float *selfX;
     int32_t *cnt; float lam;
     DropArgs dr;
     float w_in, w_add;
     int32_t wt;
 };
+static_assert(sizeof(SpmmArgs) == 376, "SpmmArgs: a new field changes the kernel-argument loads of every k_spmm instantiation");
+static inline float adam_rbc2(float c, int adam_math) { return (adam_math & LGCN_ADAM_MATH_SHORT) ? 1.0f / c : 0.f; }
+int lgcn_adam_math_initial();
 
 enum { M_SPARSE = 1, M_ADDG = 2, M_ADAM = 4, M_ADDSELF = 8, M_WTS = 16 };
 
@@ -133,6 +137,7 @@
     const long long *src; int32_t n_src; int64_t stride; int32_t P;
     float *params, *m, *v, *grad_out;
     float step_size, bc2_sqrt, w1, beta2, omb2, eps;
+    float rbc2;
 };
 void lgcn_gate_adam_launch(const GateAdamArgs &a, hipStream_t st);
 
diff --git a/graph-and-sequential-recommendation-systems_amd/csrc/lgcn_mf.hip b/graph-and-sequential-recommendation-systems_amd/csrc/lgcn_mf.hip
--- a/graph-and-sequential-recommendation-systems_amd/csrc/lgcn_mf.hip
+++ b/graph-and-sequential-recommendation-systems_amd/csrc/lgcn_mf.hip
@@ -10,6 +10,7 @@
     int64_t bm_words;
     int64_t step;
     int flip;
+    int adam_math;
 };
 
 template <int CTRL> __device__ __forceinline__ float mf_add_dpp(float v) {
@@ -93,6 +94,7 @@
     int64_t n_vec;
     const float *terms; float *loss_out; int32_t B; float decay;
     float step_size, bc2_sqrt, w1, beta2, omb2, eps;
+    float rbc2;
 };
 
 __device__ __forceinline__ void mf_reduce_loss_wave(const MfAdamArgs &a, int lane) {
@@ -134,9 +136,9 @@
         }
         m = m + a.w1 * (g - m);
         v = v * a.beta2 + (a.omb2 * g) * g;
-        f32x4 denom;
-#pragma unroll
-        for (int k = 0; k < 4; k++) denom[k] = sqrtf(v[k]) / a.bc2_sqrt + a.eps;
+        float vs[4] = {v[0], v[1], v[2], v[3]}, ds[4];
+        adam_denom<4>(vs, ds, a.bc2_sqrt, a.rbc2, a.eps);
+        const f32x4 denom = {ds[0], ds[1], ds[2], ds[3]};
         p = p - a.step_size * (m / denom);
         *reinterpret_cast<f32x4 *>(a.P + 4 * i) = p;
         *reinterpret_cast<f32x4 *>(a.M + 4 * i) = m;
@@ -155,6 +157,8 @@
     lgcn_mf *x = new (std::nothrow) lgcn_mf();
     if (!x) { lgcn_set_error("lgcn_mf_create: out of host memory"); return 4; }
     x->c = c; x->N = (int64_t)c.n_users + c.m_items; x->bm_words = (x->N + 31) / 32; x->step = 0; x->flip = 0;
+    x->adam_math = lgcn_adam_math_initial();
+    if (x->adam_math < 0) { delete x; lgcn_set_error("lgcn_mf_create: LGCN_ADAM_MATH must be 0 or 1 (LGCN_ADAM_MATH_* bits)"); return 3; }
     *out = x;
     return 0;
 }
@@ -163,6 +167,12 @@
 extern "C" int64_t lgcn_mf_get_step(const lgcn_mf *mf) { return mf ? mf->step : -1; }
 extern "C" void lgcn_mf_set_step(lgcn_mf *mf, int64_t step) { if (mf) mf->step = step; }
 extern "C" void lgcn_mf_set_lr(lgcn_mf *mf, double lr) { if (mf) mf->c.lr = lr; }
+extern "C" int lgcn_mf_set_adam_math(lgcn_mf *mf, int bits) {
+    if (bits & ~LGCN_ADAM_MATH_SHORT) { lgcn_set_error("lgcn_mf_set_adam_math: unknown adam_math bits (LGCN_ADAM_MATH_SHORT)"); return 3; }
+    if (!mf) { lgcn_set_error("lgcn_mf_set_adam_math: null context"); return 3; }
+    mf->adam_math = bits;
+    return 0;
+}
 
 static int mf_check_batch(const lgcn_mf *x, const void *u, const void *p, const void *n, const void *loss_out, int32_t B, const char *who) {
     char buf[160];
@@ -182,7 +192,7 @@
     MfAdamArgs a{};
     a.P = c.E0; a.M = c.adam_m; a.V = c.adam_v; a.G64 = (long long *)c.G64; a.bitmap = bm; a.stale_bitmap = stale; a.bitmap_words = x->bm_words;
     a.n_vec = x->N * (c.d / 4); a.terms = c.terms; a.loss_out = loss_out; a.B = B; a.decay = c.decay;
-    a.step_size = (float)(c.lr / bc1); a.bc2_sqrt = (float)sqrt(bc2);
+    a.step_size = (float)(c.lr / bc1); a.bc2_sqrt = (float)sqrt(bc2); a.rbc2 = adam_rbc2(a.bc2_sqrt, x->adam_math);
     a.w1 = (float)(1.0 - c.beta1); a.beta2 = (float)c.beta2; a.omb2 = (float)(1.0 - c.beta2); a.eps = (float)c.eps;
     int64_t blocks = (a.n_vec + 255) / 256;
     if (blocks > MF_ADAM_BLOCKS_MAX) blocks = MF_ADAM_BLOCKS_MAX;
diff --git a/graph-and-sequential-recommendation-systems_amd/csrc/lgcn_train.cpp b/graph-and-sequential-recommendation-systems_amd/csrc/lgcn_train.cpp
--- a/graph-and-sequential-recommendation-systems_amd/csrc/lgcn_train.cpp
+++ b/graph-and-sequential-recommendation-systems_amd/csrc/lgcn_train.cpp
@@ -48,6 +48,7 @@
     int32_t ib_score; const float *ib_logq;
     int32_t ib_mix;
     int32_t store_policy, wt_adam, wt_fwd;
+    int32_t adam_math;
     int32_t hn_m; uint64_t hn_seed; int32_t *hn_sel, *hn_out;
     float au_gamma; void *au_ws; int32_t au_cap;
 };
@@ -58,6 +59,15 @@
     const char *e = getenv("LGCN_STORE_POLICY");
     if (!e) return LGCN_STORE_POLICY_DEFAULT;
     if (e[0] < '0' || e[0] > '0' + (LGCN_STORE_ADAM | LGCN_STORE_XLAST) || e[1] != '\0') return -1;
+    return e[0] - '0';
+}
+#ifndef LGCN_ADAM_MATH_DEFAULT
+#define LGCN_ADAM_MATH_DEFAULT 0
+#endif
+int lgcn_adam_math_initial() {
+    const char *e = getenv("LGCN_ADAM_MATH");
+    if (!e) return LGCN_ADAM_MATH_DEFAULT;
+    if (e[0] < '0' || e[0] > '0' + LGCN_ADAM_MATH_SHORT || e[1] != '\0') return -1;
     return e[0] - '0';
 }
 int64_t lgcn_fold_segment_steps() {
@@ -102,8 +112,11 @@
     if (c.reg_ego && (gate || smooth)) { lgcn_set_error("lgcn_ctx_create: reg_ego (upstream's L2 term) is defined for the default model only, not with the optional branches"); return 3; }
     const int policy = store_policy_initial();
     if (policy < 0) { lgcn_set_error("lgcn_ctx_create: LGCN_STORE_POLICY must be one of 0, 1, 2, 3 (LGCN_STORE_* bits)"); return 3; }
+    const int adam_math = lgcn_adam_math_initial();
+    if (adam_math < 0) { lgcn_set_error("lgcn_ctx_create: LGCN_ADAM_MATH must be 0 or 1 (LGCN_ADAM_MATH_* bits)"); return 3; }
     lgcn_ctx *x = new (std::nothrow) lgcn_ctx;
     if (!x) { lgcn_set_error("out of memory"); return 4; }
+    x->adam_math = adam_math;
     x->store_policy = policy; x->wt_adam = 0; x->wt_fwd = 0;
     x->c = c; x->step = 0; x->N = c.graph->n_rows; x->cnt = nullptr; x->colsum = nullptr;
     x->drop_keep = 1.f; x->drop_seed = 0; x->dr = DropArgs{};
@@ -214,6 +227,20 @@
     if (launch_out) { launch_out[0] = ctx ? ctx->wt_adam : 0; launch_out[1] = ctx ? ctx->wt_fwd : 0; }
     return ctx ? ctx->store_policy : store_policy_initial();
 }
+extern "C" int lgcn_ctx_set_adam_math(lgcn_ctx *ctx, int bits) {
+    if (bits & ~LGCN_ADAM_MATH_SHORT) { lgcn_set_error("lgcn_ctx_set_adam_math: unknown adam_math bits (LGCN_ADAM_MATH_SHORT)"); return 3; }
+    if (!ctx) { lgcn_set_error("lgcn_ctx_set_adam_math: null context"); return 3; }
+    ctx->adam_math = bits;
+    return 0;
+}
+extern "C" int lgcn_ctx_get_adam_math(const lgcn_ctx *ctx) { return ctx ? ctx->adam_math : lgcn_adam_math_initial(); }
+extern "C" int lgcn_ctx_copy_shadow(const lgcn_ctx *ctx, void *dst_host, int64_t n) {
+    if (!ctx || !dst_host) { lgcn_set_error("lgcn_ctx_copy_shadow: null argument"); return 3; }
+    if (!ctx->e0b || n < 0 || n > ctx->N * ctx->c.d) { lgcn_set_error("lgcn_ctx_copy_shadow: the context keeps no bf16 shadow of that size"); return 3; }
+    HIP_OK(hipDeviceSynchronize());
+    HIP_OK(hipMemcpy(dst_host, ctx->e0b, sizeof(uint16_t) * (size_t)n, hipMemcpyDeviceToHost));
+    return 0;
+}
 extern "C" int lgcn_ctx_copy_arrivals(const lgcn_ctx *ctx, int32_t *dst_host, int64_t n) {
     if (!ctx || !dst_host) { lgcn_set_error("lgcn_ctx_copy_arrivals: null argument"); return 3; }
     if (ctx->variant || n < 0 || n > ctx->N) { lgcn_set_error("lgcn_ctx_copy_arrivals: the context has no arrival array of that size"); return 3; }
@@ -646,7 +673,7 @@
         x->e0b_fresh = a.Pb != nullptr || a.Pq != nullptr;
         if (x->store_policy & LGCN_STORE_ADAM) a.wt = LGCN_STORE_ARG_MV | ((a.Pb || a.Pq) ? LGCN_STORE_ARG_P : 0);
         x->wt_adam = a.wt;
-        a.step_size = (float)(c.lr / bc1); a.bc2_sqrt = (float)sqrt(bc2);
+        a.step_size = (float)(c.lr / bc1); a.bc2_sqrt = (float)sqrt(bc2); a.rbc2 = adam_rbc2(a.bc2_sqrt, x->adam_math);
         a.w1 = (float)(1.0 - c.beta1); a.beta2 = (float)c.beta2; a.omb2 = (float)(1.0 - c.beta2); a.eps = (float)c.eps;
         if (!first && fused_finish) {
             a.clear = 1; a.terms = c.terms; a.gathered = gathered; a.loss_out = loss_out;
@@ -687,7 +714,7 @@
         ga.P = x->gate_P;
         ga.params = c.gate_params; ga.m = c.gate_adam_m; ga.v = c.gate_adam_v; ga.grad_out = c.gate_grad;
         const double bc1 = 1.0 - pow(c.beta1, (double)x->step), bc2 = 1.0 - pow(c.beta2, (double)x->step);
-        ga.step_size = (float)(c.lr / bc1); ga.bc2_sqrt = (float)sqrt(bc2);
+        ga.step_size = (float)(c.lr / bc1); ga.bc2_sqrt = (float)sqrt(bc2); ga.rbc2 = adam_rbc2(ga.bc2_sqrt, x->adam_math);
         ga.w1 = (float)(1.0 - c.beta1); ga.beta2 = (float)c.beta2; ga.omb2 = (float)(1.0 - c.beta2); ga.eps = (float)c.eps;
         lgcn_gate_adam_launch(ga, st);
     }
diff --git a/graph-and-sequential-recommendation-systems_amd/model.py b/graph-and-sequential-recommendation-systems_amd/model.py
--- a/graph-and-sequential-recommendation-systems_amd/model.py
+++ b/graph-and-sequential-recommendation-systems_amd/model.py
@@ -750,6 +750,8 @@
             out.append(('lgcn_ctx_set_fold_g32', (0,)))
         if self.config.get('store_policy') is not None:
             out.append(('lgcn_ctx_set_store_policy', (int(self.config['store_policy']),)))
+        if self.config.get('adam_math') is not None:
+            out.append(('lgcn_ctx_set_adam_math', (int(self.config['adam_math']),)))
         return out
 
     def _dense_last(self, batch):
@@ -1138,7 +1140,10 @@
         self._step_workspace(st, 2 * max_batch)
         cfg = self._fill_step_config(_lib.MfConfig(), st, max_batch)
         cfg.m_items = self.m_items
-        st['ctx'] = self._create_ctx('lgcn_mf_create', cfg, [('lgcn_mf_set_step', (old_step,))])
+        setters = [('lgcn_mf_set_step', (old_step,))]
+        if self.config.get('adam_math') is not None:
+            setters.append(('lgcn_mf_set_adam_math', (int(self.config['adam_math']),)))
+        st['ctx'] = self._create_ctx('lgcn_mf_create', cfg, setters)
         st['max_batch'], st['table_ptr'] = max_batch, self._table.data_ptr()
 
     def propagated_table(self):
diff --git a/include/lgcn_hip.h b/include/lgcn_hip.h
--- a/include/lgcn_hip.h
+++ b/include/lgcn_hip.h
@@ -190,6 +190,13 @@
 #define LGCN_STORE_ARG_P 2
 #define LGCN_STORE_ARG_Y 4
 int lgcn_ctx_get_store_policy(const lgcn_ctx *ctx, int32_t *launch_out);
+
+#define LGCN_ADAM_MATH_SHORT 1
+int lgcn_ctx_set_adam_math(lgcn_ctx *ctx, int bits);
+int lgcn_ctx_get_adam_math(const lgcn_ctx *ctx);
+int lgcn_ctx_copy_shadow(const lgcn_ctx *ctx, void *dst_host, int64_t n);
+int lgcn_adam_denom_probe(int what, int adam_math, const float *c, int32_t n_c, float eps, uint32_t x_first, uint64_t n_x,
+                          uint64_t *out_host, void *stream);
 int lgcn_slot_multiplicity(const int32_t *users, const int32_t *pos, const int32_t *neg, int64_t T, int32_t B,
                            int32_t n_users, int64_t N, uint16_t *mult_out, void *stream);
 
@@ -301,6 +308,7 @@
 int64_t lgcn_mf_get_step(const lgcn_mf *mf);
 void lgcn_mf_set_step(lgcn_mf *mf, int64_t step);
 void lgcn_mf_set_lr(lgcn_mf *mf, double lr);
+int lgcn_mf_set_adam_math(lgcn_mf *mf, int bits);
 
 int lgcn_mf_train_step(lgcn_mf *mf, const int32_t *users, const int32_t *pos, const int32_t *neg,
                        int32_t B, float *loss_out, void *stream);
```

Measured after the change: 8927 steps/s, median of 6. About the same (+0.6%).
